# facebookresearch/fast3r

Hardware: AMD Instinct MI355X
Metric: views/sec (512^2, ViT-L) single forward pass at N=320 (higher is better)
Workload: dtype fp16

## Files before the change

fast3r_amd/csrc/f3r_gemm.hip:

```cpp
#include <stdlib.h>

#include "f3r_common.h"
#include "f3r_gemm_epi.h"

namespace {

constexpr int BM = 128, BN = 128, BK = 64, NT = 256;
constexpr int TILE_ELEMS = 128 * 64;
constexpr int GEMM_LDS_BYTES = 2 * 2 * TILE_ELEMS * 2;

__device__ __forceinline__ int swz(int row, int chunk) { return row * 64 + ((chunk ^ ((row >> 1) & 7)) << 3); }

struct ConvRow {
  int b, oy, ox;
  bool ok;
};

template <class T, int A_MODE, int EPI, int GLDS>
__global__ __launch_bounds__(NT, 2) void gemm_kernel(const f3r_gemm_args p) {
  extern __shared__ __attribute__((aligned(16))) uint16_t smem[];
  uint16_t* As = smem;
  uint16_t* Ws = smem + 2 * TILE_ELEMS;

  const int tid = threadIdx.x;
  const int lane = tid & 63;
  const int wid = __builtin_amdgcn_readfirstlane(tid >> 6);
  const int wm = wid >> 1, wn = wid & 1;

  const int n_tiles_n = (p.N + BN - 1) / BN;
  const int64_t n_tiles_m = (p.M + BM - 1) / BM;
  const int64_t n_wg = n_tiles_m * n_tiles_n;
  int64_t wg = blockIdx.x;
  {
    const int64_t q = n_wg / 8, r = n_wg % 8;
    const int64_t xcd = wg % 8, idx = wg / 8;
    wg = (xcd < r ? xcd * (q + 1) : r * (q + 1) + (xcd - r) * q) + idx;
  }
  constexpr int GM = 8;
  const int64_t per_group = (int64_t)GM * n_tiles_n;
  const int64_t grp = wg / per_group;
  const int64_t first_m = grp * GM;
  const int gm = (int)((n_tiles_m - first_m) < GM ? (n_tiles_m - first_m) : GM);
  const int64_t rem_ = wg - grp * per_group;
  const int tn = (int)(rem_ / gm);
  const int64_t tm = first_m + rem_ % gm;
  const int64_t m0 = tm * BM;
  const int n0 = tn * BN;

  const int sc = tid & 7;
  const int sr0 = tid >> 3;
  const uint16_t* Ag = (const uint16_t*)p.A;
  const uint16_t* Wg = (const uint16_t*)p.W;

  ConvRow cr[4];
  int64_t a_row_off[4];
  bool a_row_ok[4];
  bool w_row_ok[4];
  int64_t w_row_off[4];
#pragma unroll
  for (int i = 0; i < 4; ++i) {
    const int64_t m = m0 + sr0 + 32 * i;
    a_row_ok[i] = m < p.M;
    if (A_MODE == F3R_A_PLAIN) {
      a_row_off[i] = m * p.lda;
    } else {
      const int64_t per_img = (int64_t)p.conv_OH * p.conv_OW;
      const int64_t mm = a_row_ok[i] ? m : 0;
      cr[i].b = (int)(mm / per_img);
      const int rem = (int)(mm % per_img);
      cr[i].oy = rem / p.conv_OW;
      cr[i].ox = rem % p.conv_OW;
      cr[i].ok = a_row_ok[i];
      a_row_off[i] = 0;
    }
    const int n = n0 + sr0 + 32 * i;
    w_row_ok[i] = n < p.N;
    w_row_off[i] = (int64_t)n * p.Kpad;
  }

  const int nseg = p.split == F3R_SPLIT_NONE ? 1 : (p.split == F3R_SPLIT_W2 ? 2 : 3);
  const int Kpad1 = p.split == F3R_SPLIT_NONE ? p.Kpad : p.Kpad / 2;
  const int nk1 = Kpad1 / BK;
  const int nk = nseg * nk1;
  const int cpad_tiles = (A_MODE == F3R_A_CONV3X3) ? ((p.conv_C + 63) / 64) : 1;
  const uint16_t* Alo = (const uint16_t*)p.A_lo;

  u32x4 ra[4], rw[4];
  auto load_tile = [&](int kt_all) {
    const int seg = kt_all / nk1;
    const int kt = kt_all - seg * nk1;
    const uint16_t* Ag = (seg == 2) ? Alo : (const uint16_t*)p.A;
    if (A_MODE == F3R_A_PLAIN) {
      const int k = kt * BK + sc * 8;
      const bool kok = (k + 8) <= p.K;
#pragma unroll
      for (int i = 0; i < 4; ++i) {
        u32x4 v = {0u, 0u, 0u, 0u};
        if (a_row_ok[i] && kok) v = *(const u32x4*)(Ag + a_row_off[i] + k);
        ra[i] = v;
      }
    } else {
      const int tap = kt / cpad_tiles;
      const int ci = (kt - tap * cpad_tiles) * 64 + sc * 8;
      const int dy = tap / 3 - 1, dx = tap % 3 - 1;
      const bool cok = ci < p.conv_C;
#pragma unroll
      for (int i = 0; i < 4; ++i) {
        const int iy = cr[i].oy * p.conv_stride + dy;
        const int ix = cr[i].ox * p.conv_stride + dx;
        u32x4 v = {0u, 0u, 0u, 0u};
        if (cr[i].ok && cok && iy >= 0 && iy < p.conv_H && ix >= 0 && ix < p.conv_W) {
          const int64_t off = (((int64_t)cr[i].b * p.conv_H + iy) * p.conv_W + ix) * p.conv_C + ci;
          v = *(const u32x4*)(Ag + off);
          if (p.a_relu) {
            v[0] = relu_pk(v[0]);
            v[1] = relu_pk(v[1]);
            v[2] = relu_pk(v[2]);
            v[3] = relu_pk(v[3]);
          }
        }
        ra[i] = v;
      }
    }
    const int kw = (seg == 1 ? Kpad1 : 0) + kt * BK + sc * 8;
#pragma unroll
    for (int i = 0; i < 4; ++i) {
      u32x4 v = {0u, 0u, 0u, 0u};
      if (w_row_ok[i]) v = *(const u32x4*)(Wg + w_row_off[i] + kw);
      rw[i] = v;
    }
  };
  auto store_tile = [&](int buf) {
    uint16_t* a = As + buf * TILE_ELEMS;
    uint16_t* w = Ws + buf * TILE_ELEMS;
#pragma unroll
    for (int i = 0; i < 4; ++i) {
      const int r = sr0 + 32 * i;
      *(u32x4*)(a + swz(r, sc)) = ra[i];
      *(u32x4*)(w + swz(r, sc)) = rw[i];
    }
  };

  float4v acc[4][4];
#pragma unroll
  for (int i = 0; i < 4; ++i)
#pragma unroll
    for (int j = 0; j < 4; ++j) acc[i][j] = float4v{0.f, 0.f, 0.f, 0.f};

  const int Dq_ = p.qkv_dq ? p.qkv_dq : p.N / 3;
  const bool swap_roles = (EPI == F3R_EPI_QKV) && (n0 + wn * 64 >= Dq_ + (p.N - Dq_) / 2);

  const int fr = lane & 15;
  const int fg = lane >> 4;

  const int offA = (swap_roles ? 0 : 2 * TILE_ELEMS);
  const int offB = (swap_roles ? 2 * TILE_ELEMS : 0);
  const int rowA = (swap_roles ? wm : wn) * 64 + fr;
  const int rowB = (swap_roles ? wn : wm) * 64 + fr;

  auto compute = [&](int buf) {
    const uint16_t* ta = smem + offA + buf * TILE_ELEMS;
    const uint16_t* tb = smem + offB + buf * TILE_ELEMS;
#pragma unroll
    for (int ks = 0; ks < 2; ++ks) {
      typename T::vec8 fa[4], fb[4];
#pragma unroll
      for (int f = 0; f < 4; ++f) {
        fa[f] = as_vec8<T>(*(const u32x4*)(ta + swz(rowA + f * 16, ks * 4 + fg)));
        fb[f] = as_vec8<T>(*(const u32x4*)(tb + swz(rowB + f * 16, ks * 4 + fg)));
      }
#pragma unroll
      for (int i = 0; i < 4; ++i)
#pragma unroll
        for (int j = 0; j < 4; ++j) acc[i][j] = T::mfma16(fa[i], fb[j], acc[i][j]);
    }
  };

  if constexpr (GLDS == 1) {
    typedef __attribute__((address_space(3))) void* lds_ptr_t;
    typedef const __attribute__((address_space(1))) void* glb_ptr_t;
    const int lrow = lane >> 3, pch = lane & 7;
    const uint16_t* asrc[4];
    const uint16_t* wsrc[4];
#pragma unroll
    for (int i = 0; i < 4; ++i) {
      const int r = (wid * 4 + i) * 8 + lrow;
      const int lch = pch ^ ((r >> 1) & 7);
      int64_t m = m0 + r;
      if (m >= p.M) m = p.M - 1;
      int n = n0 + r;
      if (n >= p.N) n = p.N - 1;
      asrc[i] = Ag + m * p.lda + lch * 8;
      wsrc[i] = Wg + (int64_t)n * p.Kpad + lch * 8;
    }
    const int64_t alo_delta = Alo ? (Alo - Ag) : 0;
    auto dma_tile = [&](int kt_all, int buf) {
      const int seg = kt_all / nk1;
      const int kt = kt_all - seg * nk1;
      const int64_t ka = (seg == 2 ? alo_delta : 0) + (int64_t)kt * BK;
      const int kw = (seg == 1 ? Kpad1 : 0) + kt * BK;
#pragma unroll
      for (int i = 0; i < 4; ++i) {
        uint16_t* la = As + buf * TILE_ELEMS + (wid * 4 + i) * 8 * 64;
        uint16_t* lw = Ws + buf * TILE_ELEMS + (wid * 4 + i) * 8 * 64;
        __builtin_amdgcn_global_load_lds((glb_ptr_t)(asrc[i] + ka), (lds_ptr_t)la, 16, 0, 0);
        __builtin_amdgcn_global_load_lds((glb_ptr_t)(wsrc[i] + kw), (lds_ptr_t)lw, 16, 0, 0);
      }
    };
    dma_tile(0, 0);
    __syncthreads();
    int cur = 0;
    for (int kt = 0; kt < nk; ++kt) {
      if (kt + 1 < nk) dma_tile(kt + 1, cur ^ 1);
      compute(cur);
      __syncthreads();
      cur ^= 1;
    }
  } else {
    load_tile(0);
    store_tile(0);
    __syncthreads();
    int cur = 0;
    for (int kt = 0; kt < nk; ++kt) {
      const bool more = (kt + 1) < nk;
      if (more) load_tile(kt + 1);
      compute(cur);
      if (more) store_tile(cur ^ 1);
      __syncthreads();
      cur ^= 1;
    }
  }

  const int64_t m_base = m0 + wm * 64;
  const int n_base = n0 + wn * 64;
  if (swap_roles) gemm_epilogue_vt<T, GemmFragLayout<4, 4, 4, 4>, true>(p, &acc[0][0], m_base, n_base, lane);
  else gemm_epilogue_default<T, EPI, GemmFragLayout<4, 4, 4, 4>, true>(p, &acc[0][0], m_base, n_base, lane);
}

template <class T, int A_MODE, int EPI, int GLDS>
int launch(const f3r_gemm_args& a, hipStream_t stream) {
  static bool attr_set = false;
  auto kern = gemm_kernel<T, A_MODE, EPI, GLDS>;
  if (!attr_set) {
    (void)hipFuncSetAttribute((const void*)kern, hipFuncAttributeMaxDynamicSharedMemorySize, GEMM_LDS_BYTES);
    attr_set = true;
  }
  const int64_t tiles = ((a.M + BM - 1) / BM) * ((a.N + BN - 1) / BN);
  if (tiles <= 0) return F3R_OK;
  F3R_REQUIRE(tiles < (1ll << 31), "f3r_gemm: grid too large");
  hipLaunchKernelGGL(kern, dim3((unsigned)tiles), dim3(NT), GEMM_LDS_BYTES, stream, a);
  return f3r_check_launch("f3r_gemm");
}

template <class T>
int dispatch(const f3r_gemm_args& a, hipStream_t stream) {
  if (a.a_mode == F3R_A_CONV3X3) return launch<T, F3R_A_CONV3X3, F3R_EPI_GENERIC, 0>(a, stream);
  const int Kpad1 = a.split ? a.Kpad / 2 : a.Kpad;
  const bool glds = a.K == Kpad1 && a.M > 0;
  switch (a.epi) {
    case F3R_EPI_GENERIC: return glds ? launch<T, F3R_A_PLAIN, F3R_EPI_GENERIC, 1>(a, stream) : launch<T, F3R_A_PLAIN, F3R_EPI_GENERIC, 0>(a, stream);
    case F3R_EPI_QKV: return glds ? launch<T, F3R_A_PLAIN, F3R_EPI_QKV, 1>(a, stream) : launch<T, F3R_A_PLAIN, F3R_EPI_QKV, 0>(a, stream);
    case F3R_EPI_CONVT: return launch<T, F3R_A_PLAIN, F3R_EPI_CONVT, 0>(a, stream);
  }
  f3r_set_error("f3r_gemm: bad epi %d", a.epi);
  return F3R_ERR_ARG;
}

inline bool al16(const void* p) { return (((uintptr_t)p) & 15) == 0; }
inline bool al8(const void* p) { return (((uintptr_t)p) & 7) == 0; }

}

extern "C" int f3r_gemm(const f3r_gemm_args* args, f3r_stream_t stream) {
  F3R_REQUIRE(args != nullptr, "f3r_gemm: null args");
  const f3r_gemm_args& a = *args;
  F3R_REQUIRE(a.A && a.W, "f3r_gemm: null operand");
  F3R_REQUIRE(a.M >= 0 && a.N > 0, "f3r_gemm: bad M/N (%lld, %d)", (long long)a.M, a.N);
  F3R_REQUIRE(a.split >= F3R_SPLIT_NONE && a.split <= F3R_SPLIT_X3F8, "f3r_gemm: bad split %d", a.split);
  if (a.split == F3R_SPLIT_W2F8) {
    F3R_REQUIRE(al16(a.A) && al16(a.W) && a.w_scale && (((uintptr_t)a.w_scale) & 3) == 0, "f3r_gemm: W2F8 needs 16-byte aligned A / W and w_scale");
    F3R_REQUIRE(a.K > 0 && a.K % 128 == 0 && a.Kpad == a.K, "f3r_gemm: W2F8 needs K = Kpad, a multiple of 128 (got %d / %d)", a.K, a.Kpad);
    F3R_REQUIRE(a.lda % 8 == 0 && a.lda * 2 >= (int64_t)a.K * 3, "f3r_gemm: W2F8 rows are [K fp16 | K fp8]: lda %lld must be >= 3 K / 2", (long long)a.lda);
    F3R_REQUIRE(a.epi != F3R_EPI_GENERIC || a.out_f32 || a.out_lp, "f3r_gemm: no output");
    F3R_REQUIRE(!a.out_f8 && !a.out_relu_f8 && !a.fin_w, "f3r_gemm: W2F8 launches write one output (no out_f8 / out_relu_f8 / fin_w)");
    F3R_REQUIRE((a.kernel_sel >= 0 && a.kernel_sel <= 7) || a.kernel_sel == 9, "f3r_gemm: bad kernel_sel %d", a.kernel_sel);
    F3R_REQUIRE(a.dtype == F3R_F16, "f3r_gemm: W2F8 corrects fp16 planes only (dtype %d)", a.dtype);
    F3R_REQUIRE(a.act >= F3R_ACT_NONE && a.act <= F3R_ACT_RELU, "f3r_gemm: bad act %d", a.act);
    F3R_REQUIRE(a.N % 4 == 0 && (!a.bias || al16(a.bias)), "f3r_gemm: N %d must be a multiple of 4, bias 16-byte aligned", a.N);
    if (a.epi == F3R_EPI_GENERIC) {
      F3R_REQUIRE(!a.out_f32 || (al16(a.out_f32) && a.ldo_f32 % 4 == 0 && a.ldo_f32 >= a.N), "f3r_gemm: out_f32 alignment/ld");
      F3R_REQUIRE(!a.out_lp || (al16(a.out_lp) && a.ldo_lp % 8 == 0 && a.ldo_lp >= a.N), "f3r_gemm: out_lp alignment/ld");
      F3R_REQUIRE(!a.res_f32 || (al16(a.res_f32) && a.ldr_f32 % 4 == 0 && a.ldr_f32 >= a.N), "f3r_gemm: res_f32 alignment/ld");
    }
    const char* why = "";
    if (a.epi == F3R_EPI_QKV) {
      F3R_REQUIRE(a.qkv_dq != 0 || a.N % 3 == 0, "f3r_gemm: QKV with three equal parts needs N %% 3 == 0 (got %d)", a.N);
      {
        const int Dq = a.qkv_dq ? a.qkv_dq : a.N / 3;
        F3R_REQUIRE(Dq > 0 && Dq % 64 == 0 && a.N > Dq && (a.N - Dq) % 128 == 0, "f3r_gemm: QKV parts must be whole 64-wide heads (N %d, q %d)", a.N, Dq);
      }
      F3R_REQUIRE(a.q && a.k && a.vt && a.W_aux && al16(a.W_aux) && a.seq_len > 0 && a.M % a.seq_len == 0 && a.ldvt >= a.seq_len && a.act == F3R_ACT_NONE,
                  "f3r_gemm: W2F8 QKV needs q, k, vt, W_aux (16-byte aligned), seq_len dividing M, no activation");
      if (a.rope_cos) F3R_REQUIRE(a.rope_sin && a.rope_w > 0 && al16(a.rope_cos) && al16(a.rope_sin), "f3r_gemm: RoPE tables");
      if (!f3r_gemm_asm_qkv_eligible(a, &why)) {
        f3r_set_error("f3r_gemm: split W2F8 QKV but the launch is not eligible for the hand-scheduled kernel: %s", why);
        return F3R_ERR_UNSUPPORTED;
      }
      return f3r_gemm_asm_qkv_launch(a, (hipStream_t)stream);
    }
    if (!f3r_gemm_asm_f8_eligible(a, &why)) {
      f3r_set_error("f3r_gemm: split W2F8 (fp8 low plane) but the launch is not eligible for the hand-scheduled kernel: %s", why);
      return F3R_ERR_UNSUPPORTED;
    }
    return f3r_gemm_asm_f8_launch(a, (hipStream_t)stream);
  }
  F3R_REQUIRE(a.epi == F3R_EPI_GENERIC || (!a.out_f8 && !a.out_relu_f8 && !a.fin_w), "f3r_gemm: out_f8 / out_relu_f8 / fin_w need the generic epilogue (epi %d)", a.epi);
  const int planes = a.split ? 2 : 1;
  F3R_REQUIRE(a.Kpad > 0 && a.Kpad % (64 * planes) == 0, "f3r_gemm: Kpad %d must be a positive multiple of %d", a.Kpad, 64 * planes);
  const int Kpad1 = a.Kpad / planes;
  F3R_REQUIRE((a.split != F3R_SPLIT_X3 && a.split != F3R_SPLIT_X3F8) || (a.A_lo && al16(a.A_lo) && !a.a_relu), "f3r_gemm: X3 / X3F8 split needs A_lo (16-byte aligned) and no a_relu");
  if (a.split == F3R_SPLIT_X3F8)
    F3R_REQUIRE(a.a_mode == F3R_A_CONV3X3 && a.dtype == F3R_F16 && a.conv_C % 128 == 0 && a.w_scale && (((uintptr_t)a.w_scale) & 3) == 0,
                "f3r_gemm: X3F8 needs a 3x3 convolution with conv_C %% 128 == 0 (got %d), fp16 planes and w_scale", a.conv_C);
  F3R_REQUIRE((a.kernel_sel >= 0 && a.kernel_sel <= 7) || a.kernel_sel == 9 || a.kernel_sel >= 16, "f3r_gemm: bad kernel_sel %d", a.kernel_sel);
  F3R_REQUIRE(a.N % 4 == 0, "f3r_gemm: N %d must be a multiple of 4", a.N);
  F3R_REQUIRE(al16(a.A) && al16(a.W), "f3r_gemm: A/W must be 16-byte aligned");
  F3R_REQUIRE(a.dtype == F3R_F16 || a.dtype == F3R_BF16, "f3r_gemm: bad dtype %d", a.dtype);
  if (a.a_mode == F3R_A_PLAIN) {
    F3R_REQUIRE(a.K > 0 && a.K % 8 == 0 && a.K <= Kpad1, "f3r_gemm: K %d must be a multiple of 8 and <= Kpad", a.K);
    F3R_REQUIRE(a.lda % 8 == 0 && a.lda >= a.K, "f3r_gemm: lda %lld must be a multiple of 8 and >= K", (long long)a.lda);
  } else if (a.a_mode == F3R_A_CONV3X3) {
    F3R_REQUIRE(a.conv_C > 0 && a.conv_C % 8 == 0, "f3r_gemm: conv_C %d must be a multiple of 8", a.conv_C);
    F3R_REQUIRE(Kpad1 == 9 * ((a.conv_C + 63) / 64) * 64, "f3r_gemm: conv Kpad %d != 9*roundup(C,64) per plane", a.Kpad);
    F3R_REQUIRE(a.epi == F3R_EPI_GENERIC, "f3r_gemm: conv3x3 supports only the generic epilogue");
    F3R_REQUIRE(a.conv_stride == 1 || a.conv_stride == 2, "f3r_gemm: conv stride %d", a.conv_stride);
    F3R_REQUIRE(a.conv_OH == (a.conv_H + 2 - 3) / a.conv_stride + 1 && a.conv_OW == (a.conv_W + 2 - 3) / a.conv_stride + 1,
                "f3r_gemm: conv output dims inconsistent");
    F3R_REQUIRE(a.conv_OH > 0 && a.conv_OW > 0 && a.M % ((int64_t)a.conv_OH * a.conv_OW) == 0, "f3r_gemm: conv M not a multiple of OH*OW");
  } else {
    f3r_set_error("f3r_gemm: bad a_mode %d", a.a_mode);
    return F3R_ERR_ARG;
  }
  if (a.epi == F3R_EPI_GENERIC) {
    F3R_REQUIRE(a.out_f32 || a.out_lp || a.fin_w, "f3r_gemm: no output");
    F3R_REQUIRE(!a.out_f32 || (al16(a.out_f32) && a.ldo_f32 % 4 == 0 && a.ldo_f32 >= a.N), "f3r_gemm: out_f32 alignment/ld");
    F3R_REQUIRE(!a.out_lp || (al8(a.out_lp) && a.ldo_lp % 4 == 0 && a.ldo_lp >= a.N), "f3r_gemm: out_lp alignment/ld");
    F3R_REQUIRE((!a.out_f8 && !a.out_relu_f8) || (a.dtype == F3R_F16 && a.N % 8 == 0 && al8(a.out_f8) && al8(a.out_relu_f8) && !a.out_lp_f8),
                "f3r_gemm: out_f8 / out_relu_f8 need fp16, N %% 8 == 0 and 8-byte aligned buffers");
    if (a.fin_w) {
      F3R_REQUIRE(a.fin_b && a.fin_pts && al16(a.fin_w) && (a.fin_n_out == 3 || a.fin_n_out == 4) && (a.fin_n_out == 4 || !a.fin_conf),
                  "f3r_gemm: fin_w needs fin_b, fin_pts, a 16-byte aligned [4][N] weight and fin_n_out 3 or 4 (a confidence output needs 4)");
      F3R_REQUIRE(a.fin_depth_mode >= 0 && a.fin_depth_mode <= 2 && (a.fin_conf_mode == 0 || a.fin_conf_mode == 1), "f3r_gemm: bad fin_depth_mode / fin_conf_mode");
      F3R_REQUIRE(!a.out_f32 && !a.out_relu && !a.out_f8 && !a.out_relu_f8 && !a.res_lp && !a.res_f32 && !a.rowadd,
                  "f3r_gemm: the fused head tail writes fin_pts / fin_conf only");
    }
    F3R_REQUIRE(!a.res_f32 || (al16(a.res_f32) && a.ldr_f32 % 4 == 0), "f3r_gemm: res_f32 alignment/ld");
    F3R_REQUIRE(!a.res_lp || (al8(a.res_lp) && a.ldr_lp % 4 == 0), "f3r_gemm: res_lp alignment/ld");
    F3R_REQUIRE(!a.res_lp2 || (al8(a.res_lp2) && a.ldr_lp2 % 4 == 0), "f3r_gemm: res_lp2 alignment/ld");
    F3R_REQUIRE((!a.res_lp_lo || (a.res_lp && al8(a.res_lp_lo))) && (!a.res_lp2_lo || (a.res_lp2 && al8(a.res_lp2_lo))), "f3r_gemm: low residual planes need their high planes");
    F3R_REQUIRE((!a.out_lp_lo || (a.out_lp && al8(a.out_lp_lo))) && (!a.out_relu || (al8(a.out_relu) && a.ldo_lp % 4 == 0 && a.ldo_lp >= a.N)) &&
                (!a.out_relu_lo || (a.out_relu && al8(a.out_relu_lo))), "f3r_gemm: out_lp_lo / out_relu alignment");
    F3R_REQUIRE(!a.rowadd || (al16(a.rowadd) && a.rowadd_div > 0), "f3r_gemm: rowadd alignment/div");
    const int64_t ld_max = 1ll << 26;
    F3R_REQUIRE((!a.out_f32 || a.ldo_f32 < ld_max) && (!a.out_lp || a.ldo_lp < ld_max) && (!a.res_f32 || (a.ldr_f32 >= 0 && a.ldr_f32 < ld_max)) &&
                (!a.res_lp || (a.ldr_lp >= 0 && a.ldr_lp < ld_max)) && (!a.res_lp2 || (a.ldr_lp2 >= 0 && a.ldr_lp2 < ld_max)), "f3r_gemm: row strides must be < 2^26 elements");
    F3R_REQUIRE(!a.bias || al16(a.bias), "f3r_gemm: bias alignment");
  } else if (a.epi == F3R_EPI_QKV) {
    const int Dq = a.qkv_dq ? a.qkv_dq : a.N / 3;
    F3R_REQUIRE(a.qkv_dq != 0 || a.N % 3 == 0, "f3r_gemm: QKV with three equal parts needs N %% 3 == 0 (got %d)", a.N);
    F3R_REQUIRE(Dq > 0 && Dq % 64 == 0 && a.N > Dq && (a.N - Dq) % 128 == 0, "f3r_gemm: QKV parts must be whole 64-wide heads (N %d, q %d)", a.N, Dq);
    F3R_REQUIRE(a.q && a.k && a.vt && al8(a.q) && al8(a.k) && al8(a.vt), "f3r_gemm: QKV outputs null/misaligned");
    F3R_REQUIRE(a.seq_len > 0 && a.M % a.seq_len == 0 && a.ldvt >= a.seq_len, "f3r_gemm: QKV seq_len/ldvt");
    F3R_REQUIRE(a.act == F3R_ACT_NONE, "f3r_gemm: QKV has no activation");
    F3R_REQUIRE(!a.bias || al16(a.bias), "f3r_gemm: bias alignment");
    if (a.rope_cos) F3R_REQUIRE(a.rope_sin && a.rope_w > 0 && al16(a.rope_cos) && al16(a.rope_sin), "f3r_gemm: RoPE tables");
  } else if (a.epi == F3R_EPI_CONVT) {
    F3R_REQUIRE(a.out_lp && al8(a.out_lp), "f3r_gemm: CONVT needs out_lp");
    F3R_REQUIRE(a.ct_s > 0 && a.ct_cout > 0 && a.ct_cout % 4 == 0 && a.N == a.ct_s * a.ct_s * a.ct_cout, "f3r_gemm: CONVT N != s*s*cout");
    F3R_REQUIRE(a.ct_h > 0 && a.ct_w > 0 && a.M % ((int64_t)a.ct_h * a.ct_w) == 0, "f3r_gemm: CONVT M not a multiple of h*w");
    F3R_REQUIRE(!a.bias || al16(a.bias), "f3r_gemm: bias alignment");
  }
  hipStream_t s = (hipStream_t)stream;
  if (a.kernel_sel >= 16) return f3r_gemm256_lab(a, s);
  if (a.split == F3R_SPLIT_X3F8 || a.fin_w) {
    if (!f3r_gemm256_eligible(a)) {
      f3r_set_error("f3r_gemm: split X3F8 / fin_w but the launch is not eligible for the 256-tile kernel (conv_C %% 64 (X3F8: 128) == 0, "
                    "N %% 128 == 0 (fin_w: N == 128), operand below 4 GiB)");
      return F3R_ERR_UNSUPPORTED;
    }
    return f3r_gemm256_launch(a, s, 1);
  }
  if (a.kernel_sel == 6 || a.kernel_sel == 0 || a.kernel_sel == 9) {
    const char* why = "";
    if (a.epi == F3R_EPI_QKV && f3r_gemm_asm_qkv_eligible(a, &why) && (a.kernel_sel == 6 || a.kernel_sel == 9 || f3r_gemm_asm_preferred((a.M / 256) * (a.N / 3 / 256))))
      return f3r_gemm_asm_qkv_launch(a, s);
    const bool ok = a.epi != F3R_EPI_QKV && f3r_gemm_asm_eligible(a, &why);
    if ((a.kernel_sel == 6 || a.kernel_sel == 9) && !ok) {
      f3r_set_error("f3r_gemm: kernel_sel 6 (hand-scheduled kernel) but the launch is not eligible: %s", why);
      return F3R_ERR_UNSUPPORTED;
    }
    if (ok && (a.kernel_sel == 6 || a.kernel_sel == 9 || f3r_gemm_asm_preferred((a.M / 256) * (a.N / 256)))) return f3r_gemm_asm_launch(a, s);
  }
  const int sel = a.kernel_sel == 7 ? 0 : a.kernel_sel;
  if (sel >= 2) F3R_REQUIRE(f3r_gemm256_eligible(a), "f3r_gemm: kernel_sel %d but the shape is not eligible for the 256-tile kernel", sel);
  if (sel >= 2 || (sel == 0 && f3r_gemm256_eligible(a) && f3r_gemm256_preferred(a))) return f3r_gemm256_launch(a, s, sel != 3);
  return a.dtype == F3R_F16 ? dispatch<F16>(a, s) : dispatch<BF16>(a, s);
}
```

fast3r_amd/csrc/f3r_gemm256.hip:

```cpp
#include "f3r_gemm256_impl.h"

int f3r_gemm256_run_bf16(const f3r_gemm_args& a, hipStream_t stream, int stagger);
int f3r_gemm256_run_conv_f8_fin(const f3r_gemm_args& a, hipStream_t stream);

bool f3r_gemm256_eligible(const f3r_gemm_args& a) {
  if (a.N % 128 != 0) return false;
  if (a.epi == F3R_EPI_QKV) {
    const int Dq = a.qkv_dq ? a.qkv_dq : a.N / 3;
    if (Dq % 256 != 0 || ((a.N - Dq) / 2) % 256 != 0) return false;
  }
  const int Kpad1 = a.split ? a.Kpad / 2 : a.Kpad;
  if (Kpad1 % 64 != 0) return false;
  if (a.a_mode == F3R_A_PLAIN) {
    if (a.K != Kpad1) return false;
    if ((int64_t)256 * a.lda * 2 >= (1ll << 32)) return false;
  } else {
    if (a.a_relu || a.conv_C % 64 != 0) return false;
    if (a.M / ((int64_t)a.conv_OH * a.conv_OW) * a.conv_H * a.conv_W * a.conv_C * 2 >= (1ll << 32)) return false;
    if (a.split == F3R_SPLIT_X3F8 && (a.conv_C % 128 != 0 || a.dtype != F3R_F16)) return false;
  }
  if (a.split == F3R_SPLIT_X3F8 && a.a_mode != F3R_A_CONV3X3) return false;
  if (a.fin_w && (a.a_mode != F3R_A_CONV3X3 || a.N != 128 || a.epi != F3R_EPI_GENERIC)) return false;
  if ((int64_t)256 * a.Kpad * 2 >= (1ll << 32)) return false;
  const int add = gemm_additive_pattern(a);
  if (add == F3R_ADD_UNSUPPORTED || (add != F3R_ADD_NONE && a.act != F3R_ACT_NONE)) return false;
  if (add != F3R_ADD_NONE && a.epi != F3R_EPI_GENERIC) return false;
  if (a.a_mode == F3R_A_CONV3X3 ? (add == F3R_ADD_RES_F32 || add == F3R_ADD_ROWADD) : add == F3R_ADD_RES_LP) return false;
  return true;
}

bool f3r_gemm256_preferred(const f3r_gemm_args& a) { return score_256(a, tile_halves(a)) >= score_128(a); }

int f3r_gemm256_launch(const f3r_gemm_args& a, hipStream_t stream, int stagger) {
  const int64_t tiles = ((a.M + BM - 1) / BM) * ((a.N + 127) / 128);
  if (tiles <= 0) return F3R_OK;
  F3R_REQUIRE(tiles < (1ll << 31), "f3r_gemm: grid too large");
  if (a.split == F3R_SPLIT_X3F8 || a.fin_w) return f3r_gemm256_run_conv_f8_fin(a, stream);
  return a.dtype == F3R_F16 ? dispatch256<F16>(a, stream, stagger) : f3r_gemm256_run_bf16(a, stream, stagger);
}
```

fast3r_amd/csrc/f3r_gemm256_f8.hip:

```cpp
#include <cstdlib>

#include "f3r_gemm256_impl.h"

int f3r_gemm256_run_conv_f8_fin(const f3r_gemm_args& a, hipStream_t stream) {
  const bool f8 = a.split == F3R_SPLIT_X3F8;
  const int add = gemm_additive_pattern(a);
  if (a.fin_w) {
#ifdef F3R_CONV_ABLATIONS
    if (f8) {
      static const char* ab = getenv("F3R_CONV_ABLATE");
      switch (ab ? atoi(ab) : 0) {
#define F3R_ABL(n) case n: return launch256<F16, F3R_A_CONV3X3, F3R_EPI_GENERIC, 1, F3R_ADD_NONE, 1, true, true, false, n>(a, stream);
        F3R_ABL(1) F3R_ABL(1024) F3R_ABL(2048) F3R_ABL(2) F3R_ABL(4) F3R_ABL(3) F3R_ABL(7)
#undef F3R_ABL
      }
    }
#endif
    if (a.dtype == F3R_BF16) return launch256<BF16, F3R_A_CONV3X3, F3R_EPI_GENERIC, 1, F3R_ADD_NONE, 1, false, true>(a, stream);
    if (f8 && a.kernel_sel == 5) return launch256<F16, F3R_A_CONV3X3, F3R_EPI_GENERIC, 1, F3R_ADD_NONE, 1, true, true, true>(a, stream);
    return f8 ? launch256<F16, F3R_A_CONV3X3, F3R_EPI_GENERIC, 1, F3R_ADD_NONE, 1, true, true>(a, stream)
              : launch256<F16, F3R_A_CONV3X3, F3R_EPI_GENERIC, 1, F3R_ADD_NONE, 1, false, true>(a, stream);
  }
  const int nh = tile_halves(a);
  if (add == F3R_ADD_RES_LP)
    return nh == 2 ? launch256<F16, F3R_A_CONV3X3, F3R_EPI_GENERIC, 1, F3R_ADD_RES_LP, 2, true>(a, stream)
                   : launch256<F16, F3R_A_CONV3X3, F3R_EPI_GENERIC, 1, F3R_ADD_RES_LP, 1, true>(a, stream);
  return nh == 2 ? launch256<F16, F3R_A_CONV3X3, F3R_EPI_GENERIC, 1, F3R_ADD_NONE, 2, true>(a, stream)
                 : launch256<F16, F3R_A_CONV3X3, F3R_EPI_GENERIC, 1, F3R_ADD_NONE, 1, true>(a, stream);
}
```

fast3r_amd/csrc/f3r_gemm256_impl.h:

```cpp
#pragma once
#include <atomic>

#include "f3r_common.h"
#include "f3r_gemm_epi.h"


namespace {

constexpr int BM = 256, BK = 64, NT = 512;
constexpr int HT = 128 * 64;
template <int NH> struct TileCfg {
  static constexpr int BN = 128 * NH;
  static constexpr int BUF = (2 + NH) * HT;
  static constexpr int NBUF = NH == 2 ? 2 : 3;
  static constexpr int TAB_ENTRIES = 512;
  static constexpr int LDS_BYTES = NBUF * BUF * 2 + TAB_ENTRIES * 16;
};

inline int f3r_num_cus() {
  constexpr int MAXD = 64;
  static std::atomic<int> cache[MAXD];
  int dev = 0;
  if (hipGetDevice(&dev) != hipSuccess) dev = 0;
  if (dev >= 0 && dev < MAXD) {
    const int c = cache[dev].load(std::memory_order_relaxed);
    if (c) return c;
  }
  int cu = 0;
  if (hipDeviceGetAttribute(&cu, hipDeviceAttributeMultiprocessorCount, dev) != hipSuccess || cu < 8) cu = 256;
  const int n = cu / 8 * 8;
  if (dev >= 0 && dev < MAXD) cache[dev].store(n, std::memory_order_relaxed);
  return n;
}

typedef __attribute__((address_space(3))) void* lds_ptr_t;
typedef const __attribute__((address_space(1))) void* glb_ptr_t;

template <int V>
struct IC {
  static constexpr int value = V;
};

#define F3R_VMCNT(n) __builtin_amdgcn_s_waitcnt(0x0F70 | (n))
#define F3R_LGKMCNT0() __builtin_amdgcn_s_waitcnt(0xC07F)

template <class T, int A_MODE, int EPI, bool SWAP, int STAGGER, int ADDSRC, int NH = 2, int LAB = 0, bool F8 = false, bool FIN = false, bool MERGED = false>
__device__ __forceinline__ void gemm256_body(const f3r_gemm_args& p, uint16_t* smem, const int64_t m0_tile, const int n0_tile, const bool first = true,
                                             const bool has_next = false, const int64_t m0_next = 0, const int n0_next = 0) {
  constexpr int BUF = TileCfg<NH>::BUF;
  int64_t m0 = m0_tile;
  int n0 = n0_tile;
  const int tid = threadIdx.x;
  const int lane = tid & 63;
  const int wid = __builtin_amdgcn_readfirstlane(tid >> 6);
  const int wm = wid >> 2, wn = wid & 3;
  const int fr = lane & 15, fg = lane >> 4;
  constexpr bool PAIRED = EPI != F3R_EPI_QKV && (ADDSRC == F3R_ADD_NONE || ADDSRC == F3R_ADD_RES_LP);
  static_assert(!(PAIRED && SWAP), "swapped roles exist only in the QKV role");
  auto w_key = [](int r) { return PAIRED ? (((r >> 1) & 1) | (((r >> 3) & 3) << 1)) : ((r >> 1) & 7); };
  uint64_t stamp[5] = {0, 0, 0, 0, 0};
  if (LAB & 128) stamp[0] = __builtin_amdgcn_s_memtime();
  if ((LAB & (256 | 512)) && blockIdx.x < 256) {
    const int PH = (LAB & 512) ? 4 : 2;
    const int phase = (blockIdx.x >> 3) & (PH - 1);
    const int n = phase * (p.Kpad / BK) * (4 / PH);
    for (int i = 0; i < n; ++i) __builtin_amdgcn_s_sleep(15);
  }

  const int nseg = p.split == F3R_SPLIT_NONE ? 1 : (p.split == F3R_SPLIT_W2 ? 2 : 3);
  const int Kpad1 = p.split == F3R_SPLIT_NONE ? p.Kpad : p.Kpad / 2;
  const int nk1 = Kpad1 / BK;
  const int nk8 = nk1 / 2;
  const int nk = F8 ? nk1 + 2 * nk8 : nseg * nk1;
  const int ctiles = A_MODE == F3R_A_CONV3X3 ? p.conv_C / 64 : 1;
  const int ctiles8 = A_MODE == F3R_A_CONV3X3 ? p.conv_C / 128 : 1;
  static_assert(!F8 || (A_MODE == F3R_A_CONV3X3 && !SWAP), "fp8 correction segments: convolutions only");
  static_assert(!FIN || (NH == 1 && EPI == F3R_EPI_GENERIC && ADDSRC == 0 && !SWAP), "fused head tail: 256 x 128 tiles, no additive terms");

  uint32_t a_off[2][2], w_off[2][2];
  uint32_t a_msk[2][2];
  const char* const Ab = (const char*)p.A;
  const char* const Alo = (const char*)p.A_lo;
  const uint32_t a_bytes = A_MODE == F3R_A_CONV3X3 ? (uint32_t)(p.M / ((int64_t)p.conv_OH * p.conv_OW) * p.conv_H * p.conv_W * p.conv_C * 2) : 0u;
  const char* Wb = nullptr;
  uint32_t wsc[NH][2];
  auto setup_tile = [&](int64_t tm0, int tn0) {
  m0 = tm0;
  n0 = tn0;
  Wb = (const char*)p.W + (int64_t)n0 * p.Kpad * 2;
  if constexpr (F8) {
#pragma unroll
    for (int h = 0; h < NH; ++h)
#pragma unroll
      for (int nf = 0; nf < 2; ++nf) {
        int n = n0 + h * 128 + (wid & 3) * 32 + (PAIRED ? (fr >> 2) * 8 + (fr & 3) + nf * 4 : fr + nf * 16);
        if (n >= p.N) n = p.N - 1;
        wsc[h][nf] = p.w_scale[n];
      }
  }
#pragma unroll
  for (int h = 0; h < 2; ++h)
#pragma unroll
    for (int i = 0; i < 2; ++i) {
      const int r = (wid * 2 + i) * 8 + (lane >> 3);
      const int lc = (lane & 7) ^ ((r >> 1) & 7);
      int n = n0 + (h < NH ? h : 0) * 128 + r;
      if (n >= p.N) n = p.N - 1;
      w_off[h][i] = (uint32_t)(((int64_t)(n - n0) * p.Kpad + ((lane & 7) ^ w_key(r)) * 8) * 2);
      int64_t m = m0 + h * 128 + r;
      if (A_MODE == F3R_A_PLAIN) {
        if (m >= p.M) m = p.M - 1;
        a_off[h][i] = (uint32_t)(((m - m0) * p.lda + lc * 8) * 2);
        a_msk[h][i] = 0;
      } else {
        const bool ok = m < p.M;
        const int64_t per_img = (int64_t)p.conv_OH * p.conv_OW;
        const int64_t mm = ok ? m : 0;
        const int b = (int)(mm / per_img);
        const int rem = (int)(mm % per_img);
        const int oy = rem / p.conv_OW, ox = rem - oy * p.conv_OW;
        const int cy = oy * p.conv_stride, cx = ox * p.conv_stride;
        a_off[h][i] = (uint32_t)(((((int64_t)b * p.conv_H + cy) * p.conv_W + cx) * p.conv_C + lc * 8) * 2);
        uint32_t msk = 0;
#pragma unroll
        for (int tap = 0; tap < 9; ++tap) {
          const int iy = cy + tap / 3 - 1, ix = cx + tap % 3 - 1;
          if (!(ok && iy >= 0 && iy < p.conv_H && ix >= 0 && ix < p.conv_W)) msk |= 1u << tap;
        }
        a_msk[h][i] = msk;
      }
    }
  };
  setup_tile(m0_tile, n0_tile);

  constexpr bool TAB = A_MODE == F3R_A_CONV3X3;
  const int pix = TAB ? p.conv_C * 2 : 0;
  uint32_t* const tab = (uint32_t*)(smem + TileCfg<NH>::NBUF * BUF);
  if (TAB && first) {
    for (int t = tid; t < nk; t += NT) {
      int delta, meta, wso;
      if (!F8 || t < nk1) {
        const int seg = F8 ? 0 : t / nk1, kk = t - seg * nk1, tapn = kk / ctiles, ct = kk - tapn * ctiles;
        delta = ((tapn / 3 - 1) * p.conv_W + (tapn % 3 - 1)) * pix + ct * 128;
        meta = tapn | ((!F8 && seg == 2) ? 16 : 0);
        wso = ((seg == 1 ? Kpad1 : 0) + kk * BK) * 2;
      } else {
        const int u = t - nk1, s8 = u / nk8, kk = u - s8 * nk8, tapn = kk / ctiles8, ct = kk - tapn * ctiles8;
        delta = ((tapn / 3 - 1) * p.conv_W + (tapn % 3 - 1)) * pix + (s8 == 1 ? p.conv_C : 0) + ct * 128;
        meta = tapn | 16;
        wso = (s8 + 2) * Kpad1 + kk * 128;
      }
      *(u32x4*)(tab + t * 4) = u32x4{(uint32_t)delta, (uint32_t)meta, (uint32_t)wso, 0u};
    }
    __syncthreads();
  }
  u32x4 ea = {0u, 0u, 0u, 0u}, ew = ea;
  int a_seg = 0, a_kk = 0, a_t = 0;
  int w_seg = 0, w_kk = 0, w_t = 0;
  auto fetch = [&]() {
    if constexpr (TAB) {
      ea = *(const u32x4*)(tab + a_t * 4);
      ew = *(const u32x4*)(tab + w_t * 4);
    }
  };
  bool dry = false;
  auto a_advance = [&]() {
    if (a_t + 1 < nk) {
      ++a_t;
      if constexpr (!TAB) {
        ++a_kk;
        if (a_kk == nk1) { a_kk = 0; ++a_seg; }
      }
    }
  };
  auto w_advance = [&]() {
    if (w_t + 1 < nk) {
      ++w_t;
      if constexpr (!TAB) {
        ++w_kk;
        if (w_kk == nk1) { w_kk = 0; ++w_seg; }
      }
    }
  };
  bool in_loop = false;
  auto issue_a = [&](int h, int buf) {
    if (dry) return;
    if ((LAB & (1 | 2048)) && in_loop) return;
    const char* plane = (!TAB && a_seg == 2) ? Alo : Ab;
    uint16_t* dst = smem + buf * BUF + h * HT + wid * 2 * 8 * 64;
    if (A_MODE == F3R_A_PLAIN) {
      const char* base = plane + (m0 * p.lda + (int64_t)a_kk * BK) * 2;
      if (LAB & 32) {
        const __amdgpu_buffer_rsrc_t rs = __builtin_amdgcn_make_buffer_rsrc((void*)(plane + m0 * p.lda * 2), 0, 0x7fffffff, 0x00020000);
#pragma unroll
        for (int i = 0; i < 2; ++i)
          __builtin_amdgcn_raw_ptr_buffer_load_lds(rs, (lds_ptr_t)(dst + i * 8 * 64), 16, (int)a_off[h][i], a_kk * BK * 2, 0, 0);
        return;
      }
#pragma unroll
      for (int i = 0; i < 2; ++i)
        __builtin_amdgcn_global_load_lds((glb_ptr_t)(base + a_off[h][i]), (lds_ptr_t)(dst + i * 8 * 64), 16, 0, 0);
    } else {
      const int a_delta = __builtin_amdgcn_readfirstlane((int)ea[0]);
      const int meta = __builtin_amdgcn_readfirstlane((int)ea[1]);
      const int a_tap = meta & 15;
      const char* pl = (meta & 16) ? Alo : Ab;
      const __amdgpu_buffer_rsrc_t rs = __builtin_amdgcn_make_buffer_rsrc((void*)pl, 0, a_bytes, 0x00020000);
#pragma unroll
      for (int i = 0; i < 2; ++i) {
        const int32_t inv = ((int32_t)(a_msk[h][i] << (31 - a_tap))) >> 31;
        const uint32_t vo = (a_off[h][i] + (uint32_t)a_delta) | (uint32_t)inv;
        __builtin_amdgcn_raw_ptr_buffer_load_lds(rs, (lds_ptr_t)(dst + i * 8 * 64), 16, (int)vo, 0, 0, 0);
      }
    }
  };
  auto issue_w = [&](int h, int buf) {
    if (dry) return;
    if ((LAB & (1 | 1024)) && in_loop) return;
    uint16_t* dst = smem + buf * BUF + (2 + h) * HT + wid * 2 * 8 * 64;
    if constexpr (TAB) {
      const int w_soff = __builtin_amdgcn_readfirstlane((int)ew[2]);
      const __amdgpu_buffer_rsrc_t rs = __builtin_amdgcn_make_buffer_rsrc((void*)Wb, 0, 0x7fffffff, 0x00020000);
#pragma unroll
      for (int i = 0; i < 2; ++i)
        __builtin_amdgcn_raw_ptr_buffer_load_lds(rs, (lds_ptr_t)(dst + i * 8 * 64), 16, (int)w_off[h][i], w_soff, 0, 0);
      return;
    }
    const char* base = Wb + ((int64_t)(w_seg == 1 ? Kpad1 : 0) + (int64_t)w_kk * BK) * 2;
    if (LAB & 32) {
      const __amdgpu_buffer_rsrc_t rs = __builtin_amdgcn_make_buffer_rsrc((void*)Wb, 0, 0x7fffffff, 0x00020000);
#pragma unroll
      for (int i = 0; i < 2; ++i)
        __builtin_amdgcn_raw_ptr_buffer_load_lds(rs, (lds_ptr_t)(dst + i * 8 * 64), 16, (int)w_off[h][i], ((w_seg == 1 ? Kpad1 : 0) + w_kk * BK) * 2, 0, 0);
      return;
    }
#pragma unroll
    for (int i = 0; i < 2; ++i)
      __builtin_amdgcn_global_load_lds((glb_ptr_t)(base + w_off[h][i]), (lds_ptr_t)(dst + i * 8 * 64), 16, 0, 0);
  };

  const int sw = (fr >> 1) & 7;
  const int w_row = wn * 32 + (PAIRED ? (fr >> 2) * 8 + (fr & 3) : fr);
  int a_rd[2], w_rd[2];
#pragma unroll
  for (int ks = 0; ks < 2; ++ks) {
    a_rd[ks] = (wm * 64 + fr) * 64 + (((ks * 4 + fg) ^ sw) << 3);
    w_rd[ks] = w_row * 64 + (((ks * 4 + fg) ^ w_key(w_row)) << 3);
  }

  float4v acc[16 * NH];
  typename T::vec8 fa0[2][4], fa1[2][4], fw[2][2];
  typedef uint32_t u32x8 __attribute__((ext_vector_type(8)));
  typedef int i32x8 __attribute__((ext_vector_type(8)));
  u32x8 ga0[4], ga1[4], gw[2];

  auto read_a = [&](auto e8, auto which, int buf, int mh) {
    if ((LAB & 2) && in_loop) return;
    if constexpr (decltype(e8)::value) {
      auto& g = decltype(which)::value ? ga1 : ga0;
#pragma unroll
      for (int mf = 0; mf < 4; ++mf) {
        const u32x4 c0 = *(const u32x4*)(smem + buf * BUF + mh * HT + a_rd[0] + mf * 16 * 64);
        const u32x4 c1 = *(const u32x4*)(smem + buf * BUF + mh * HT + a_rd[1] + mf * 16 * 64);
        g[mf] = __builtin_shufflevector(c0, c1, 0, 1, 2, 3, 4, 5, 6, 7);
      }
    } else {
      auto& f = decltype(which)::value ? fa1 : fa0;
#pragma unroll
      for (int ks = 0; ks < 2; ++ks)
#pragma unroll
        for (int mf = 0; mf < 4; ++mf)
          f[ks][mf] = as_vec8<T>(*(const u32x4*)(smem + buf * BUF + mh * HT + a_rd[ks] + mf * 16 * 64));
    }
  };
  auto read_w = [&](auto e8, int buf, int nh) {
    if ((LAB & 2) && in_loop) return;
    if constexpr (decltype(e8)::value) {
#pragma unroll
      for (int nf = 0; nf < 2; ++nf) {
        const u32x4 c0 = *(const u32x4*)(smem + buf * BUF + (2 + nh) * HT + w_rd[0] + nf * (PAIRED ? 4 : 16) * 64);
        const u32x4 c1 = *(const u32x4*)(smem + buf * BUF + (2 + nh) * HT + w_rd[1] + nf * (PAIRED ? 4 : 16) * 64);
        gw[nf] = __builtin_shufflevector(c0, c1, 0, 1, 2, 3, 4, 5, 6, 7);
      }
    } else {
#pragma unroll
      for (int ks = 0; ks < 2; ++ks)
#pragma unroll
        for (int nf = 0; nf < 2; ++nf)
          fw[ks][nf] = as_vec8<T>(*(const u32x4*)(smem + buf * BUF + (2 + nh) * HT + w_rd[ks] + nf * (PAIRED ? 4 : 16) * 64));
    }
  };
  auto mma = [&](auto e8, auto which, int mh, int nh, int sa_shift, int sb) {
    if (LAB & 4) return;
    if constexpr (decltype(e8)::value) {
      auto& g = decltype(which)::value ? ga1 : ga0;
#pragma unroll
      for (int nf = 0; nf < 2; ++nf) {
        const int sa = (int)((wsc[nh < NH ? nh : 0][nf] >> sa_shift) & 0xffu);
#pragma unroll
        for (int mf = 0; mf < 4; ++mf) {
          const int NF = nh * 2 + nf, MF = mh * 4 + mf;
          acc[NF * 8 + MF] = __builtin_amdgcn_mfma_scale_f32_16x16x128_f8f6f4(__builtin_bit_cast(i32x8, gw[nf]), __builtin_bit_cast(i32x8, g[mf]),
                                                                              acc[NF * 8 + MF], 0, 0, 0, sa, 0, sb);
        }
      }
#pragma unroll
      for (int nf = 0; nf < 2; ++nf)
#pragma unroll
        for (int mf = 0; mf < 4; ++mf) asm volatile("" : "+v"(acc[(nh * 2 + nf) * 8 + mh * 4 + mf]));
    } else {
      auto& f = decltype(which)::value ? fa1 : fa0;
#pragma unroll
      for (int ks = 0; ks < 2; ++ks)
#pragma unroll
        for (int nf = 0; nf < 2; ++nf)
#pragma unroll
          for (int mf = 0; mf < 4; ++mf) {
            const int NF = nh * 2 + nf, MF = mh * 4 + mf;
            if (SWAP) acc[MF * (2 * NH) + NF] = T::mfma16(f[ks][mf], fw[ks][nf], acc[MF * (2 * NH) + NF]);
            else      acc[NF * 8 + MF] = T::mfma16(fw[ks][nf], f[ks][mf], acc[NF * 8 + MF]);
          }
    }
  };

#define F3R_PHASE_MMA(WHICH, MH, NH)                     \
  __builtin_amdgcn_sched_barrier(0);                     \
  __builtin_amdgcn_s_barrier();                          \
  F3R_LGKMCNT0();                                        \
  __builtin_amdgcn_sched_barrier(0);                     \
  if (!(LAB & 16)) __builtin_amdgcn_s_setprio(1);        \
  mma(e8, IC<WHICH>{}, MH, NH, sa_shift, sb);            \
  if (!(LAB & 16)) __builtin_amdgcn_s_setprio(0);        \
  __builtin_amdgcn_sched_barrier(0);                     \
  __builtin_amdgcn_s_barrier();
  auto tile = [&](auto bufc, auto e8, int sa_shift, int sb) {
    constexpr int B = decltype(bufc)::value;
    fetch();
    read_w(e8, B, 0);
    if (!(LAB & 64)) __builtin_amdgcn_sched_barrier(0);
    read_a(e8, IC<0>{}, B, 0);
    issue_a(1, B ^ 1);
    a_advance();
    if (!(LAB & 8)) F3R_VMCNT(8);
    F3R_PHASE_MMA(0, 0, 0)
    fetch();
    read_a(e8, IC<1>{}, B, 1);
    issue_w(1, B ^ 1);
    w_advance();
    if (!(LAB & 8)) F3R_VMCNT(8);
    F3R_PHASE_MMA(1, 1, 0)
    fetch();
    read_w(e8, B, 1);
    issue_a(0, B);
    F3R_PHASE_MMA(1, 1, 1)
    fetch();
    issue_w(0, B);
    if (!(LAB & 8)) F3R_VMCNT(8);
    F3R_PHASE_MMA(0, 0, 1)
  };
  auto tile1 = [&](auto bufc, auto e8, int sa_shift, int sb) {
    constexpr int B = decltype(bufc)::value;
    constexpr int B2 = (B + 2) % 3;
    fetch();
    read_w(e8, B, 0);
    if (!(LAB & 64)) __builtin_amdgcn_sched_barrier(0);
    read_a(e8, IC<0>{}, B, 0);
    issue_a(0, B2);
    issue_w(0, B2);
    w_advance();
    if (!(LAB & 8)) F3R_VMCNT(10);
    F3R_PHASE_MMA(0, 0, 0)
    read_a(e8, IC<1>{}, B, 1);
    issue_a(1, B2);
    a_advance();
    if (!(LAB & 8)) F3R_VMCNT(8);
    F3R_PHASE_MMA(1, 1, 0)
  };
#define F3R_MMA2_OPEN()                                  \
  __builtin_amdgcn_sched_barrier(0);                     \
  __builtin_amdgcn_s_barrier();                          \
  F3R_LGKMCNT0();                                        \
  __builtin_amdgcn_sched_barrier(0);                     \
  __builtin_amdgcn_s_setprio(1);
#define F3R_MMA2_ISSUE()                                 \
  __builtin_amdgcn_s_setprio(0);                         \
  __builtin_amdgcn_sched_barrier(0);
#define F3R_MMA2_CLOSE()                                 \
  __builtin_amdgcn_sched_barrier(0);                     \
  __builtin_amdgcn_s_barrier();
  auto tileM = [&](auto bufc, auto e8, int sa_shift, int sb) {
    constexpr int B = decltype(bufc)::value;
    fetch();
    read_w(e8, B, 0);
    __builtin_amdgcn_sched_barrier(0);
    read_a(e8, IC<0>{}, B, 0);
    read_a(e8, IC<1>{}, B, 1);
    issue_w(1, B ^ 1);
    w_advance();
    F3R_VMCNT(8);
    F3R_MMA2_OPEN()
    mma(e8, IC<0>{}, 0, 0, sa_shift, sb);
    mma(e8, IC<1>{}, 1, 0, sa_shift, sb);
    F3R_MMA2_ISSUE()
    F3R_MMA2_CLOSE()
    fetch();
    read_w(e8, B, 1);
    issue_a(0, B);
    issue_w(0, B);
    issue_a(1, B);
    a_advance();
    F3R_VMCNT(8);
    F3R_MMA2_OPEN()
    mma(e8, IC<1>{}, 1, 1, sa_shift, sb);
    mma(e8, IC<0>{}, 0, 1, sa_shift, sb);
    F3R_MMA2_ISSUE()
    F3R_MMA2_CLOSE()
  };
  auto tile1M = [&](auto bufc, auto e8, int sa_shift, int sb) {
    constexpr int B = decltype(bufc)::value;
    constexpr int B2 = (B + 2) % 3;
    fetch();
    read_w(e8, B, 0);
    __builtin_amdgcn_sched_barrier(0);
    read_a(e8, IC<0>{}, B, 0);
    read_a(e8, IC<1>{}, B, 1);
    issue_a(0, B2);
    issue_w(0, B2);
    w_advance();
    issue_a(1, B2);
    a_advance();
    F3R_VMCNT(6);
    F3R_MMA2_OPEN()
    mma(e8, IC<0>{}, 0, 0, sa_shift, sb);
    mma(e8, IC<1>{}, 1, 0, sa_shift, sb);
    F3R_MMA2_ISSUE()
    F3R_MMA2_CLOSE()
  };
#undef F3R_MMA2_OPEN
#undef F3R_MMA2_ISSUE
#undef F3R_MMA2_CLOSE
#undef F3R_PHASE_MMA

  typedef GemmFragLayout<2 * NH, 8, 2, 4, PAIRED> Frag;
  const int64_t m_base = m0_tile + wm * 64;
  const int n_base = n0_tile + wn * 32;
  auto opening_loads = [&]() {
    a_seg = a_kk = a_t = 0;
    w_seg = w_kk = w_t = 0;
    if constexpr (NH == 2) {
      if (!dry) fetch();
      issue_a(0, 0);
      issue_w(0, 0);
      issue_a(1, 0);
      a_advance();
      issue_w(1, 0);
      w_advance();
      if (!dry) fetch();
      issue_a(0, 1);
      issue_w(0, 1);
      if constexpr (MERGED) {
        issue_a(1, 1);
        a_advance();
      }
    } else {
      if (!dry) fetch();
      issue_a(0, 0);
      issue_w(0, 0);
      w_advance();
      issue_a(1, 0);
      a_advance();
      if (!dry) fetch();
      issue_a(0, 1);
      issue_w(0, 1);
      w_advance();
      issue_a(1, 1);
      a_advance();
    }
  };
  dry = !first;
  opening_loads();
  dry = false;
  gemm_acc_init_additive<T, Frag, ADDSRC, SWAP>(p, acc, m_base, n_base, lane);
  if (first && MERGED) {
    if constexpr (NH == 2) F3R_VMCNT(8);
    else F3R_VMCNT(6);
  } else if (first) {
    F3R_VMCNT(8);
  } else {
    F3R_VMCNT(0);
  }
  __builtin_amdgcn_s_barrier();
  if (STAGGER && wm == 1) __builtin_amdgcn_s_barrier();
  if (LAB & 128) stamp[1] = __builtin_amdgcn_s_memtime();

  typedef IC<0> E16;
  typedef IC<1> E8;
  auto T2 = [&](auto bufc, auto e8, int sa_shift, int sb) {
    if constexpr (MERGED) tileM(bufc, e8, sa_shift, sb);
    else tile(bufc, e8, sa_shift, sb);
  };
  auto T1 = [&](auto bufc, auto e8, int sa_shift, int sb) {
    if constexpr (MERGED) tile1M(bufc, e8, sa_shift, sb);
    else tile1(bufc, e8, sa_shift, sb);
  };
  const int nk16 = F8 ? nk1 : nk;
  if constexpr (NH == 2) {
    if (LAB) {
      tile(IC<0>{}, E16{}, 0, 0);
      if (nk > 1) tile(IC<1>{}, E16{}, 0, 0);
      in_loop = true;
    }
    for (int t = LAB ? 2 : 0; t < nk16; t += 2) {
      T2(IC<0>{}, E16{}, 0, 0);
      if (t + 1 < nk16) T2(IC<1>{}, E16{}, 0, 0);
    }
    if constexpr (F8) {
      for (int t = 0; t < nk1; t += 2) {
        T2(IC<0>{}, E8{}, t >= nk8 ? 8 : 0, t >= nk8 ? 115 : 127);
        T2(IC<1>{}, E8{}, t + 1 >= nk8 ? 8 : 0, t + 1 >= nk8 ? 115 : 127);
      }
    }
  } else {
    if (LAB) in_loop = true;
    for (int t = 0; t < nk16; t += 3) {
      T1(IC<0>{}, E16{}, 0, 0);
      if (t + 1 < nk16) T1(IC<1>{}, E16{}, 0, 0);
      if (t + 2 < nk16) T1(IC<2>{}, E16{}, 0, 0);
    }
    if constexpr (F8) {
      for (int t = 0; t < nk1; t += 3) {
        T1(IC<0>{}, E8{}, t >= nk8 ? 8 : 0, t >= nk8 ? 115 : 127);
        T1(IC<1>{}, E8{}, t + 1 >= nk8 ? 8 : 0, t + 1 >= nk8 ? 115 : 127);
        T1(IC<2>{}, E8{}, t + 2 >= nk8 ? 8 : 0, t + 2 >= nk8 ? 115 : 127);
      }
    }
  }
  F3R_VMCNT(0);
  if (STAGGER && wm == 0) __builtin_amdgcn_s_barrier();
  if (LAB & 128) stamp[2] = __builtin_amdgcn_s_memtime();
  if (has_next) {
    setup_tile(m0_next, n0_next);
    opening_loads();
  }

  if constexpr (FIN) {
    __builtin_amdgcn_s_barrier();
    gemm_epilogue_fin<T, Frag>(p, acc, m0_tile, wm, wn, lane, tid, (float*)(smem + 2 * BUF));
  } else if (SWAP) gemm_epilogue_vt<T, Frag, false>(p, acc, m_base, n_base, lane);
  else gemm_epilogue_default<T, EPI, Frag, false>(p, acc, m_base, n_base, lane);
  if (LAB & 128) {
    __builtin_amdgcn_sched_barrier(0);
    stamp[3] = __builtin_amdgcn_s_memtime();
    F3R_VMCNT(0);
    stamp[4] = __builtin_amdgcn_s_memtime();
    if (tid == 0) {
      uint64_t* d = (uint64_t*)p.rope_cos + (int64_t)blockIdx.x * 5;
      for (int i = 0; i < 5; ++i) d[i] = stamp[i];
    }
  }
}

template <class T, int A_MODE, int EPI, int STAGGER, int ADDSRC, int NH, bool F8 = false, bool FIN = false, bool MERGED = false, int LAB = 0>
__global__ __launch_bounds__(NT, 1) void gemm256_kernel(const f3r_gemm_args p) {
  extern __shared__ __attribute__((aligned(16))) uint16_t smem[];
  constexpr int BN = TileCfg<NH>::BN;
  const int n_tiles_n = (p.N + BN - 1) / BN;
  const int64_t n_tiles_m = (p.M + BM - 1) / BM;
  const int64_t n_wg = n_tiles_m * n_tiles_n;
  auto tile_of = [&](int64_t wg, int64_t& m0, int& n0) {
    {
      const int64_t q = n_wg / 8, r = n_wg % 8;
      const int64_t xcd = wg % 8, idx = wg / 8;
      wg = (xcd < r ? xcd * (q + 1) : r * (q + 1) + (xcd - r) * q) + idx;
    }
    constexpr int GM = 8;
    const int64_t per_group = (int64_t)GM * n_tiles_n;
    const int64_t grp = wg / per_group;
    const int64_t first_m = grp * GM;
    const int gm = (int)((n_tiles_m - first_m) < GM ? (n_tiles_m - first_m) : GM);
    const int64_t rem_ = wg - grp * per_group;
    const int tn = (int)(rem_ / gm);
    const int64_t tm = first_m + rem_ % gm;
    m0 = tm * BM;
    n0 = tn * BN;
  };
  int64_t m0, m0n = 0;
  int n0, n0n = 0;
  bool first = true;
  for (int64_t v = blockIdx.x; v < n_wg; v += gridDim.x) {
    tile_of(v, m0, n0);
    const bool has_next = v + gridDim.x < n_wg;
    if (has_next) tile_of(v + gridDim.x, m0n, n0n);
    bool done = false;
    if constexpr (EPI == F3R_EPI_QKV) {
      if (n0 >= (p.qkv_dq ? p.qkv_dq + (p.N - p.qkv_dq) / 2 : 2 * (p.N / 3))) {
        gemm256_body<T, A_MODE, EPI, true, STAGGER, F3R_ADD_NONE, NH>(p, smem, m0, n0, first, has_next, m0n, n0n);
        done = true;
      }
    }
    if (!done) gemm256_body<T, A_MODE, EPI, false, STAGGER, ADDSRC, NH, LAB, F8, FIN, MERGED>(p, smem, m0, n0, first, has_next, m0n, n0n);
    first = false;
  }
}

template <class T, int A_MODE, int EPI, int STAGGER, int ADDSRC, int NH, bool F8 = false, bool FIN = false, bool MERGED = false, int LAB = 0>
int launch256(const f3r_gemm_args& a, hipStream_t stream) {
  static bool attr_set = false;
  auto kern = gemm256_kernel<T, A_MODE, EPI, STAGGER, ADDSRC, NH, F8, FIN, MERGED, LAB>;
  constexpr int LDS_BYTES = TileCfg<NH>::LDS_BYTES, BN = TileCfg<NH>::BN;
  if (!attr_set) {
    (void)hipFuncSetAttribute((const void*)kern, hipFuncAttributeMaxDynamicSharedMemorySize, LDS_BYTES);
    attr_set = true;
  }
  const int64_t tiles = ((a.M + BM - 1) / BM) * ((a.N + BN - 1) / BN);
  const int64_t grid = (a.kernel_sel == 5 || tiles <= f3r_num_cus()) ? tiles : f3r_num_cus();
  hipLaunchKernelGGL(kern, dim3((unsigned)grid), dim3(NT), LDS_BYTES, stream, a);
  return f3r_check_launch("f3r_gemm(256)");
}

inline float tile_score(int64_t tiles, int slots, float eff) {
  if (tiles <= 0) return 0.f;
  const int64_t rounds = (tiles + slots - 1) / slots;
  return eff * (float)tiles / (float)(rounds * slots);
}
inline float score_256(const f3r_gemm_args& a, int nh) {
  return tile_score(((a.M + 255) / 256) * ((a.N + 128 * nh - 1) / (128 * nh)), 256, nh == 2 ? 1.0f : 0.82f);
}
inline float score_128(const f3r_gemm_args& a) { return tile_score(((a.M + 127) / 128) * ((a.N + 127) / 128), 512, 0.72f); }

inline int tile_halves(const f3r_gemm_args& a) {
  if (a.epi == F3R_EPI_QKV) return 2;
  if (a.N % 256 != 0 || a.kernel_sel == 4) return 1;
  if (a.kernel_sel == 2 || a.kernel_sel == 3 || a.kernel_sel == 5) return 2;
  return score_256(a, 1) > score_256(a, 2) ? 1 : 2;
}

template <class T>
int dispatch256(const f3r_gemm_args& a, hipStream_t stream, int stagger) {
#define F3R_L256H(AM, EP, AD, NHV) (stagger ? launch256<T, AM, EP, 1, AD, NHV>(a, stream) : launch256<T, AM, EP, 0, AD, NHV>(a, stream))
#define F3R_L256(AM, EP, AD) (nh == 2 ? F3R_L256H(AM, EP, AD, 2) : F3R_L256H(AM, EP, AD, 1))
  const int add = gemm_additive_pattern(a);
  const int nh = tile_halves(a);
  if (a.a_mode == F3R_A_CONV3X3) return add == F3R_ADD_RES_LP ? F3R_L256(F3R_A_CONV3X3, F3R_EPI_GENERIC, F3R_ADD_RES_LP) : F3R_L256(F3R_A_CONV3X3, F3R_EPI_GENERIC, F3R_ADD_NONE);
  switch (a.epi) {
    case F3R_EPI_GENERIC:
      return add == F3R_ADD_RES_F32 ? F3R_L256(F3R_A_PLAIN, F3R_EPI_GENERIC, F3R_ADD_RES_F32)
           : add == F3R_ADD_ROWADD ? F3R_L256(F3R_A_PLAIN, F3R_EPI_GENERIC, F3R_ADD_ROWADD) : F3R_L256(F3R_A_PLAIN, F3R_EPI_GENERIC, F3R_ADD_NONE);
    case F3R_EPI_QKV: return F3R_L256H(F3R_A_PLAIN, F3R_EPI_QKV, F3R_ADD_NONE, 2);
    default: return F3R_L256(F3R_A_PLAIN, F3R_EPI_CONVT, F3R_ADD_NONE);
  }
#undef F3R_L256
#undef F3R_L256H
}

#ifdef F3R_GEMM_LAB
template <class T, int LAB>
__global__ __launch_bounds__(NT, 1) void gemm256_lab_kernel(const f3r_gemm_args p) {
  extern __shared__ __attribute__((aligned(16))) uint16_t smem[];
  constexpr int BN = 256;
  const int n_tiles_n = (p.N + BN - 1) / BN;
  const int64_t wg = blockIdx.x;
  gemm256_body<T, F3R_A_PLAIN, F3R_EPI_GENERIC, false, 1, F3R_ADD_NONE, 2, LAB>(p, smem, (wg / n_tiles_n) * BM, (int)(wg % n_tiles_n) * BN);
}
template <class T, int LAB>
int launch_lab(const f3r_gemm_args& a, hipStream_t stream) {
  auto kern = gemm256_lab_kernel<T, LAB>;
  constexpr int BN = 256, LDS_BYTES = TileCfg<2>::LDS_BYTES;
  (void)hipFuncSetAttribute((const void*)kern, hipFuncAttributeMaxDynamicSharedMemorySize, LDS_BYTES);
  const int64_t tiles = ((a.M + BM - 1) / BM) * ((a.N + BN - 1) / BN);
  hipLaunchKernelGGL(kern, dim3((unsigned)tiles), dim3(NT), LDS_BYTES, stream, a);
  return f3r_check_launch("f3r_gemm(256 lab)");
}
#endif

}
```

fast3r_amd/csrc/f3r_gemm_epi.h:

```cpp
#pragma once
#include "f3r_common.h"

template <int NF_, int MF_, int NG_, int MG_, bool PAIRED_ = false>
struct GemmFragLayout {
  static constexpr int NF = NF_, MF = MF_, NG = NG_, MG = MG_;
  static constexpr bool PAIRED = PAIRED_;
  static constexpr int LW = PAIRED_ ? 8 : 4;
  static constexpr int STEP = PAIRED_ ? 2 : 1;
  static_assert(!PAIRED_ || NG_ == 2, "paired columns: two fragments per 32-column group");
  static __device__ __forceinline__ int row(int mf) { return (mf / MG) * 128 + (mf % MG) * 16; }
  static __device__ __forceinline__ int col(int nf) { return (nf / NG) * 128 + (nf % NG) * (PAIRED_ ? 4 : 16); }
  static __device__ __forceinline__ int col_end() { return ((NF - 1) / NG) * 128 + NG * 16; }
};

__device__ __forceinline__ float gelu_erf(float x) {
  const float z = fabsf(x) * 0.70710678118654752440f;
  const float t = __builtin_amdgcn_rcpf(__builtin_fmaf(0.3275911f, z, 1.0f));
  float poly = __builtin_fmaf(1.061405429f, t, -1.453152027f);
  poly = __builtin_fmaf(poly, t, 1.421413741f);
  poly = __builtin_fmaf(poly, t, -0.284496736f);
  poly = __builtin_fmaf(poly, t, 0.254829592f);
  const float u = poly * t * __builtin_amdgcn_exp2f(-z * z * 1.44269504088896340736f);
  const float h = 0.5f * x * u;
  return x >= 0.f ? x - h : h;
}

__device__ __forceinline__ float4v gelu_erf4(float4v x) {
  float4v t, e;
#pragma unroll
  for (int i = 0; i < 4; ++i) t[i] = __builtin_amdgcn_rcpf(__builtin_fmaf(__builtin_fabsf(x[i]), 0.3275911f * 0.70710678118654752440f, 1.0f));
  float4v poly = t * (0.5f * 1.061405429f) + (0.5f * -1.453152027f);
  poly = poly * t + (0.5f * 1.421413741f);
  poly = poly * t + (0.5f * -0.284496736f);
  poly = poly * t + (0.5f * 0.254829592f);
  const float4v arg = (x * x) * (-0.5f * 1.44269504088896340736f);
#pragma unroll
  for (int i = 0; i < 4; ++i) e[i] = __builtin_amdgcn_exp2f(arg[i]);
  const float4v h = x * (poly * t * e);
  float4v r;
#pragma unroll
  for (int i = 0; i < 4; ++i) r[i] = __builtin_fmaf(x[i] + __builtin_fabsf(x[i]), 0.5f, -__builtin_fabsf(h[i]));
  return r;
}

template <class T>
__device__ __forceinline__ void store4_split(uint16_t* hi, uint16_t* lo, float4v v) {
  u32x2 o;
  o[0] = pack2<T>(v[0], v[1]);
  o[1] = pack2<T>(v[2], v[3]);
  *(u32x2*)hi = o;
  if (lo) {
    u32x2 r;
    r[0] = pack2<T>(v[0] - lo_f<T>(o[0]), v[1] - hi_f<T>(o[0]));
    r[1] = pack2<T>(v[2] - lo_f<T>(o[1]), v[3] - hi_f<T>(o[1]));
    *(u32x2*)lo = r;
  }
}

template <class T>
__device__ __forceinline__ float4v load4_lp(const uint16_t* ptr) {
  const u32x2 r = *(const u32x2*)ptr;
  return float4v{lo_f<T>(r[0]), hi_f<T>(r[0]), lo_f<T>(r[1]), hi_f<T>(r[1])};
}

template <class T, int STEP>
__device__ __forceinline__ void storeN_split(char* hi, char* lo, const float4v* v) {
  if constexpr (STEP == 1) {
    store4_split<T>((uint16_t*)hi, (uint16_t*)lo, v[0]);
  } else {
    u32x4 o;
    o[0] = pack2<T>(v[0][0], v[0][1]); o[1] = pack2<T>(v[0][2], v[0][3]);
    o[2] = pack2<T>(v[1][0], v[1][1]); o[3] = pack2<T>(v[1][2], v[1][3]);
    *(u32x4*)hi = o;
    if (lo) {
      u32x4 r;
      r[0] = pack2<T>(v[0][0] - lo_f<T>(o[0]), v[0][1] - hi_f<T>(o[0])); r[1] = pack2<T>(v[0][2] - lo_f<T>(o[1]), v[0][3] - hi_f<T>(o[1]));
      r[2] = pack2<T>(v[1][0] - lo_f<T>(o[2]), v[1][1] - hi_f<T>(o[2])); r[3] = pack2<T>(v[1][2] - lo_f<T>(o[3]), v[1][3] - hi_f<T>(o[3]));
      *(u32x4*)lo = r;
    }
  }
}
template <class T, int STEP>
__device__ __forceinline__ void loadN_lp(const char* ptr, float4v* v) {
  if constexpr (STEP == 1) {
    v[0] = load4_lp<T>((const uint16_t*)ptr);
  } else {
    const u32x4 r = *(const u32x4*)ptr;
    v[0] = float4v{lo_f<T>(r[0]), hi_f<T>(r[0]), lo_f<T>(r[1]), hi_f<T>(r[1])};
    v[1] = float4v{lo_f<T>(r[2]), hi_f<T>(r[2]), lo_f<T>(r[3]), hi_f<T>(r[3])};
  }
}

__device__ __forceinline__ uint32_t f8x4(float a, float b, float c, float d) {
  auto cl = [](float x) { return fminf(fmaxf(x, -448.f), 448.f); };
  int w = __builtin_amdgcn_cvt_pk_fp8_f32(cl(a), cl(b), 0, false);
  w = __builtin_amdgcn_cvt_pk_fp8_f32(cl(c), cl(d), w, true);
  return (uint32_t)w;
}
__device__ __forceinline__ float f16_rest(float x) { return (x - (float)(_Float16)x) * 4096.f; }
template <int STEP>
__device__ __forceinline__ void storeN_f8(char* hi8, char* lo8, const float4v* v) {
  if constexpr (STEP == 1) {
    *(uint32_t*)hi8 = f8x4(v[0][0], v[0][1], v[0][2], v[0][3]);
    *(uint32_t*)lo8 = f8x4(f16_rest(v[0][0]), f16_rest(v[0][1]), f16_rest(v[0][2]), f16_rest(v[0][3]));
  } else {
    u32x2 h, l;
    h[0] = f8x4(v[0][0], v[0][1], v[0][2], v[0][3]);
    h[1] = f8x4(v[1][0], v[1][1], v[1][2], v[1][3]);
    l[0] = f8x4(f16_rest(v[0][0]), f16_rest(v[0][1]), f16_rest(v[0][2]), f16_rest(v[0][3]));
    l[1] = f8x4(f16_rest(v[1][0]), f16_rest(v[1][1]), f16_rest(v[1][2]), f16_rest(v[1][3]));
    *(u32x2*)hi8 = h;
    *(u32x2*)lo8 = l;
  }
}

template <class T, int NF, int MB, class F>
__device__ __forceinline__ void gemm_additive_terms(const f3r_gemm_args& p, const int64_t (&mc)[MB], const int (&nbc)[NF], F&& term) {
  if (p.rowadd) {
#pragma unroll
    for (int i = 0; i < MB; ++i) {
      const float* row = p.rowadd + (mc[i] / p.rowadd_div) * (int64_t)p.N;
#pragma unroll
      for (int nf = 0; nf < NF; ++nf) term(i, nf, *(const float4v*)(row + nbc[nf]));
    }
  }
  if (p.res_f32) {
#pragma unroll
    for (int i = 0; i < MB; ++i)
#pragma unroll
      for (int nf = 0; nf < NF; ++nf) term(i, nf, *(const float4v*)(p.res_f32 + mc[i] * p.ldr_f32 + nbc[nf]));
  }
  if (p.res_lp) {
#pragma unroll
    for (int i = 0; i < MB; ++i)
#pragma unroll
      for (int nf = 0; nf < NF; ++nf) term(i, nf, load4_lp<T>((const uint16_t*)p.res_lp + mc[i] * p.ldr_lp + nbc[nf]));
    if (p.res_lp_lo) {
#pragma unroll
      for (int i = 0; i < MB; ++i)
#pragma unroll
        for (int nf = 0; nf < NF; ++nf) term(i, nf, load4_lp<T>((const uint16_t*)p.res_lp_lo + mc[i] * p.ldr_lp + nbc[nf]));
    }
  }
  if (p.res_lp2) {
#pragma unroll
    for (int i = 0; i < MB; ++i)
#pragma unroll
      for (int nf = 0; nf < NF; ++nf) term(i, nf, load4_lp<T>((const uint16_t*)p.res_lp2 + mc[i] * p.ldr_lp2 + nbc[nf]));
    if (p.res_lp2_lo) {
#pragma unroll
      for (int i = 0; i < MB; ++i)
#pragma unroll
        for (int nf = 0; nf < NF; ++nf) term(i, nf, load4_lp<T>((const uint16_t*)p.res_lp2_lo + mc[i] * p.ldr_lp2 + nbc[nf]));
    }
  }
}

enum { F3R_ADD_NONE = 0, F3R_ADD_RES_F32 = 1, F3R_ADD_ROWADD = 2, F3R_ADD_RES_LP = 3, F3R_ADD_UNSUPPORTED = -1 };

inline int gemm_additive_pattern(const f3r_gemm_args& a) {
  const int n_kinds = (a.rowadd != nullptr) + (a.res_f32 != nullptr) + (a.res_lp != nullptr || a.res_lp2 != nullptr);
  if (n_kinds == 0) return F3R_ADD_NONE;
  if (n_kinds > 1 || (a.res_lp2 && !a.res_lp)) return F3R_ADD_UNSUPPORTED;
  return a.rowadd ? F3R_ADD_ROWADD : (a.res_f32 ? F3R_ADD_RES_F32 : F3R_ADD_RES_LP);
}

template <class T, class L, int SRC, bool SWAP>
__device__ __forceinline__ void gemm_acc_init_additive(const f3r_gemm_args& p, float4v* acc, int64_t m_base, int n_base, int lane) {
  constexpr int NF = L::NF, MF = L::MF;
  const int fr = lane & 15, fg = lane >> 4;
  if (SWAP) {
#pragma unroll
    for (int nf = 0; nf < NF; ++nf) {
      const int n = n_base + L::col(nf) + fr;
      const float b = (p.bias && n < p.N) ? p.bias[n] : 0.f;
#pragma unroll
      for (int mf = 0; mf < MF; ++mf) acc[mf * NF + nf] = float4v{b, b, b, b};
    }
    return;
  }
  if (SRC != F3R_ADD_ROWADD && m_base + L::row(MF - 1) + 16 <= p.M && n_base + L::col_end() <= p.N) {
    float4v b4[NF];
#pragma unroll
    for (int nf = 0; nf < NF; ++nf)
      b4[nf] = p.bias ? *(const float4v*)((const char*)(p.bias + n_base + L::col(nf)) + (uint32_t)(fg * L::LW * 4)) : float4v{0.f, 0.f, 0.f, 0.f};
    if (SRC == F3R_ADD_NONE) {
#pragma unroll
      for (int nf = 0; nf < NF; ++nf)
#pragma unroll
        for (int mf = 0; mf < MF; ++mf) acc[nf * MF + mf] = b4[nf];
      return;
    }
    if (SRC == F3R_ADD_RES_F32) {
      const uint32_t off = (uint32_t)(fr * (int)p.ldr_f32 + fg * L::LW) * 4u;
#pragma unroll
      for (int mf = 0; mf < MF; ++mf) {
        const char* const row = (const char*)p.res_f32 + ((m_base + L::row(mf)) * p.ldr_f32 + n_base) * 4;
#pragma unroll
        for (int nf = 0; nf < NF; ++nf) acc[nf * MF + mf] = *(const float4v*)(row + L::col(nf) * 4 + off);
      }
    } else {
      const uint32_t off = (uint32_t)(fr * (int)p.ldr_lp + fg * L::LW) * 2u;
      const uint32_t off2 = (uint32_t)(fr * (int)p.ldr_lp2 + fg * L::LW) * 2u;
#pragma unroll
      for (int mf = 0; mf < MF; ++mf) {
        const int64_t ro = ((m_base + L::row(mf)) * p.ldr_lp + n_base) * 2;
#pragma unroll
        for (int nf = 0; nf < NF; nf += L::STEP) {
          float4v t[L::STEP];
          loadN_lp<T, L::STEP>((const char*)p.res_lp + ro + L::col(nf) * 2 + off, t);
#pragma unroll
          for (int q = 0; q < L::STEP; ++q) acc[(nf + q) * MF + mf] = t[q];
        }
      }
      if (p.res_lp_lo) {
#pragma unroll
        for (int mf = 0; mf < MF; ++mf) {
          const int64_t ro = ((m_base + L::row(mf)) * p.ldr_lp + n_base) * 2;
#pragma unroll
          for (int nf = 0; nf < NF; nf += L::STEP) {
            float4v t[L::STEP];
            loadN_lp<T, L::STEP>((const char*)p.res_lp_lo + ro + L::col(nf) * 2 + off, t);
#pragma unroll
            for (int q = 0; q < L::STEP; ++q) acc[(nf + q) * MF + mf] += t[q];
          }
        }
      }
      if (p.res_lp2) {
#pragma unroll
        for (int mf = 0; mf < MF; ++mf) {
          const int64_t ro = ((m_base + L::row(mf)) * p.ldr_lp2 + n_base) * 2;
#pragma unroll
          for (int nf = 0; nf < NF; nf += L::STEP) {
            float4v t[L::STEP];
            loadN_lp<T, L::STEP>((const char*)p.res_lp2 + ro + L::col(nf) * 2 + off2, t);
#pragma unroll
            for (int q = 0; q < L::STEP; ++q) acc[(nf + q) * MF + mf] += t[q];
          }
        }
        if (p.res_lp2_lo) {
#pragma unroll
          for (int mf = 0; mf < MF; ++mf) {
            const int64_t ro = ((m_base + L::row(mf)) * p.ldr_lp2 + n_base) * 2;
#pragma unroll
            for (int nf = 0; nf < NF; nf += L::STEP) {
            float4v t[L::STEP];
            loadN_lp<T, L::STEP>((const char*)p.res_lp2_lo + ro + L::col(nf) * 2 + off2, t);
#pragma unroll
            for (int q = 0; q < L::STEP; ++q) acc[(nf + q) * MF + mf] += t[q];
          }
          }
        }
      }
    }
#pragma unroll
    for (int nf = 0; nf < NF; ++nf)
#pragma unroll
      for (int mf = 0; mf < MF; ++mf) acc[nf * MF + mf] += b4[nf];
    return;
  }
  int nbc[NF];
  float4v bias4[NF];
#pragma unroll
  for (int nf = 0; nf < NF; ++nf) {
    const int nb = n_base + L::col(nf) + fg * L::LW;
    nbc[nf] = nb < p.N ? nb : p.N - 4;
    bias4[nf] = p.bias ? *(const float4v*)(p.bias + nbc[nf]) : float4v{0.f, 0.f, 0.f, 0.f};
  }
  if (SRC == F3R_ADD_NONE) {
#pragma unroll
    for (int nf = 0; nf < NF; ++nf)
#pragma unroll
      for (int mf = 0; mf < MF; ++mf) acc[nf * MF + mf] = bias4[nf];
    return;
  }
  int64_t mc[MF];
#pragma unroll
  for (int mf = 0; mf < MF; ++mf) {
    const int64_t m = m_base + L::row(mf) + fr;
    mc[mf] = m < p.M ? m : p.M - 1;
  }
  if (SRC == F3R_ADD_RES_F32) {
#pragma unroll
    for (int mf = 0; mf < MF; ++mf)
#pragma unroll
      for (int nf = 0; nf < NF; ++nf) acc[nf * MF + mf] = *(const float4v*)(p.res_f32 + mc[mf] * p.ldr_f32 + nbc[nf]);
  } else if (SRC == F3R_ADD_ROWADD) {
#pragma unroll
    for (int mf = 0; mf < MF; ++mf) {
      const float* row = p.rowadd + (mc[mf] / p.rowadd_div) * (int64_t)p.N;
#pragma unroll
      for (int nf = 0; nf < NF; ++nf) acc[nf * MF + mf] = *(const float4v*)(row + nbc[nf]);
    }
  } else {
#pragma unroll
    for (int mf = 0; mf < MF; ++mf)
#pragma unroll
      for (int nf = 0; nf < NF; ++nf) acc[nf * MF + mf] = load4_lp<T>((const uint16_t*)p.res_lp + mc[mf] * p.ldr_lp + nbc[nf]);
    if (p.res_lp_lo) {
#pragma unroll
      for (int mf = 0; mf < MF; ++mf)
#pragma unroll
        for (int nf = 0; nf < NF; ++nf) acc[nf * MF + mf] += load4_lp<T>((const uint16_t*)p.res_lp_lo + mc[mf] * p.ldr_lp + nbc[nf]);
    }
    if (p.res_lp2) {
#pragma unroll
      for (int mf = 0; mf < MF; ++mf)
#pragma unroll
        for (int nf = 0; nf < NF; ++nf) acc[nf * MF + mf] += load4_lp<T>((const uint16_t*)p.res_lp2 + mc[mf] * p.ldr_lp2 + nbc[nf]);
      if (p.res_lp2_lo) {
#pragma unroll
        for (int mf = 0; mf < MF; ++mf)
#pragma unroll
          for (int nf = 0; nf < NF; ++nf) acc[nf * MF + mf] += load4_lp<T>((const uint16_t*)p.res_lp2_lo + mc[mf] * p.ldr_lp2 + nbc[nf]);
      }
    }
  }
#pragma unroll
  for (int nf = 0; nf < NF; ++nf)
#pragma unroll
    for (int mf = 0; mf < MF; ++mf) acc[nf * MF + mf] += bias4[nf];
}

#define F3R_EPI_WAIT_LOADS() __builtin_amdgcn_s_waitcnt(0x0F70)

template <class L>
__device__ __forceinline__ bool gemm_wave_interior(const f3r_gemm_args& p, int64_t m_base, int n_base) {
  return m_base + L::row(L::MF - 1) + 16 <= p.M && n_base + L::col_end() <= p.N;
}

template <int V>
struct EpiC {
  static constexpr int value = V;
};

template <class T, class L>
__device__ __forceinline__ void gemm_epilogue_generic_interior(const f3r_gemm_args& p, const float4v* acc, int64_t m_base, int n_base, int lane) {
  constexpr int NF = L::NF, MF = L::MF;
  const int fr = lane & 15, fg = lane >> 4;
  const uint32_t off_f32 = (uint32_t)(fr * (int)p.ldo_f32 + fg * L::LW) * 4u;
  const uint32_t off_lp = (uint32_t)(fr * (int)p.ldo_lp + fg * L::LW) * 2u;
  const uint32_t off_f8 = (uint32_t)(fr * p.N * 2 + fg * L::LW);
  const bool relu = p.act == F3R_ACT_RELU;
  auto run = [&](auto act_c, auto kind_c) {
    constexpr int ACT = decltype(act_c)::value, KIND = decltype(kind_c)::value;
#pragma unroll
    for (int mf = 0; mf < MF; ++mf) {
      const int64_t mrow = m_base + L::row(mf);
      char* const bf = (KIND >= 2 && p.out_f32) ? (char*)p.out_f32 + (mrow * p.ldo_f32 + n_base) * 4 : nullptr;
      const int64_t lp_row = (mrow * p.ldo_lp + n_base) * 2;
      char* const bl = (KIND != 2 && p.out_lp) ? (char*)p.out_lp + lp_row : nullptr;
      char* const bll = ((KIND == 1 || KIND == 3) && p.out_lp_lo) ? (char*)p.out_lp_lo + lp_row : nullptr;
      char* const br = (KIND == 3 && p.out_relu) ? (char*)p.out_relu + lp_row : nullptr;
      char* const brl = (KIND == 3 && p.out_relu_lo) ? (char*)p.out_relu_lo + lp_row : nullptr;
      char* const b8 = (KIND == 3 && p.out_f8) ? (char*)p.out_f8 + (mrow * p.N * 2 + n_base) : nullptr;
      char* const br8 = (KIND == 3 && p.out_relu_f8) ? (char*)p.out_relu_f8 + (mrow * p.N * 2 + n_base) : nullptr;
#pragma unroll
      for (int nf = 0; nf < NF; nf += L::STEP) {
        float4v v[L::STEP];
#pragma unroll
        for (int q = 0; q < L::STEP; ++q) {
          v[q] = acc[(nf + q) * MF + mf];
          if (ACT == F3R_ACT_GELU) v[q] = gelu_erf4(v[q]);
          else if (relu) v[q] = float4v{fmaxf(v[q][0], 0.f), fmaxf(v[q][1], 0.f), fmaxf(v[q][2], 0.f), fmaxf(v[q][3], 0.f)};
        }
        const int cb = L::col(nf);
        if (KIND >= 2 && bf) {
#pragma unroll
          for (int q = 0; q < L::STEP; ++q) *(float4v*)(bf + (cb + q * 4) * 4 + off_f32) = v[q];
        }
        if (KIND != 2 && bl) storeN_split<T, L::STEP>(bl + cb * 2 + off_lp, (KIND == 1 || (KIND == 3 && bll)) ? bll + cb * 2 + off_lp : nullptr, v);
        if (KIND == 3 && b8) storeN_f8<L::STEP>(b8 + cb + off_f8, b8 + cb + off_f8 + p.N, v);
        if (KIND == 3 && (br || br8)) {
          float4v r[L::STEP];
#pragma unroll
          for (int q = 0; q < L::STEP; ++q) r[q] = float4v{fmaxf(v[q][0], 0.f), fmaxf(v[q][1], 0.f), fmaxf(v[q][2], 0.f), fmaxf(v[q][3], 0.f)};
          if (br) storeN_split<T, L::STEP>(br + cb * 2 + off_lp, brl ? brl + cb * 2 + off_lp : nullptr, r);
          if (br8) storeN_f8<L::STEP>(br8 + cb + off_f8, br8 + cb + off_f8 + p.N, r);
        }
      }
    }
  };
  auto by_kind = [&](auto act_c) {
    const bool f32 = p.out_f32 != nullptr, lp = p.out_lp != nullptr, lo = p.out_lp_lo != nullptr, rl = p.out_relu != nullptr || p.out_f8 != nullptr || p.out_relu_f8 != nullptr;
    if (lp && !f32 && !lo && !rl) run(act_c, EpiC<0>{});
    else if (lp && lo && !f32 && !rl) run(act_c, EpiC<1>{});
    else if (f32 && !lp && !rl) run(act_c, EpiC<2>{});
    else run(act_c, EpiC<3>{});
  };
  if (p.act == F3R_ACT_GELU) by_kind(EpiC<F3R_ACT_GELU>{});
  else by_kind(EpiC<F3R_ACT_NONE>{});
}

template <class T, class L>
__device__ __forceinline__ void gemm_epilogue_qk_interior(const f3r_gemm_args& p, const float4v* acc, int64_t m_base, int n_base, int lane) {
  constexpr int NF = L::NF, MF = L::MF, MB = 4;
  const int fr = lane & 15, fg = lane >> 4;
  const int Dq = p.qkv_dq ? p.qkv_dq : p.N / 3;
  const int Dkv = (p.N - Dq) / 2;
  const int part = n_base < Dq ? 0 : 1;
  const int Dm = part == 0 ? Dq : Dkv;
  const int col0 = part == 0 ? 0 : Dq;
  char* const dst = (char*)(part == 0 ? p.q : p.k);
  const float qs = (part == 0 && p.q_scale != 0.f) ? p.q_scale : 1.f;
  const uint32_t off = (uint32_t)(fr * Dm + fg * L::LW) * 2u;
  const uint32_t seq = (uint32_t)p.seq_len, rw = (uint32_t)(p.rope_w > 0 ? p.rope_w : 1);
#pragma unroll
  for (int mb = 0; mb < MF; mb += MB) {
    float4v c[MB][NF / 2], sn[MB][NF / 2];
    if (p.rope_cos) {
#pragma unroll
      for (int i = 0; i < MB; ++i) {
        const uint32_t m = (uint32_t)(m_base + L::row(mb + i)) + (uint32_t)fr;
        const uint32_t pos = m % seq;
        const uint32_t py = pos / rw, px = pos - py * rw;
        const uint32_t grp = m / rw;
#pragma unroll
        for (int j = 0; j < NF / 2; ++j) {
          const int h = ((n_base + L::col(2 * j)) >> 5) & 1;
          const int64_t toff = p.rope_mode == 1 ? (int64_t)grp * 32 + h * 16 : (int64_t)(h == 0 ? py : px) * 16;
          c[i][j] = *(const float4v*)(p.rope_cos + toff + fg * 4);
          sn[i][j] = *(const float4v*)(p.rope_sin + toff + fg * 4);
        }
      }
      F3R_EPI_WAIT_LOADS();
    }
#pragma unroll
    for (int i = 0; i < MB; ++i) {
      char* const row = dst + ((m_base + L::row(mb + i)) * Dm + (n_base - col0)) * 2;
      float4v v[NF];
#pragma unroll
      for (int nf = 0; nf < NF; ++nf) v[nf] = acc[nf * MF + mb + i];
      if (p.rope_cos) {
#pragma unroll
        for (int j = 0; j < NF / 2; ++j) {
          const float4v a = v[2 * j], b = v[2 * j + 1];
          v[2 * j] = a * c[i][j] - b * sn[i][j];
          v[2 * j + 1] = b * c[i][j] + a * sn[i][j];
        }
      }
#pragma unroll
      for (int nf = 0; nf < NF; ++nf) store4_split<T>((uint16_t*)(row + L::col(nf) * 2 + off), nullptr, v[nf] * qs);
    }
  }
}

template <class T, int EPI, class L, bool ADD>
__device__ __forceinline__ void gemm_epilogue_default(const f3r_gemm_args& p, const float4v* acc, int64_t m_base, int n_base, int lane) {
  constexpr int NF = L::NF, MF = L::MF;
  if constexpr (!ADD && EPI != F3R_EPI_CONVT) {
    if (gemm_wave_interior<L>(p, m_base, n_base) && p.M <= 0x7fffffffll) {
      if constexpr (EPI == F3R_EPI_GENERIC) gemm_epilogue_generic_interior<T, L>(p, acc, m_base, n_base, lane);
      else gemm_epilogue_qk_interior<T, L>(p, acc, m_base, n_base, lane);
      return;
    }
  }
  const int fr = lane & 15, fg = lane >> 4;
  constexpr int MB = 4;
  static_assert(MF % MB == 0, "MF must be a multiple of the batch");
  int nb[NF], nbc[NF];
  float4v bias4[NF];
#pragma unroll
  for (int nf = 0; nf < NF; ++nf) {
    nb[nf] = n_base + L::col(nf) + fg * L::LW;
    nbc[nf] = nb[nf] < p.N ? nb[nf] : p.N - 4;
    bias4[nf] = (ADD && p.bias) ? *(const float4v*)(p.bias + nbc[nf]) : float4v{0.f, 0.f, 0.f, 0.f};
  }
  if (ADD) F3R_EPI_WAIT_LOADS();
  if (EPI == F3R_EPI_GENERIC || EPI == F3R_EPI_CONVT) {
#pragma unroll
    for (int mb = 0; mb < MF; mb += MB) {
      int64_t m[MB], mc[MB];
#pragma unroll
      for (int i = 0; i < MB; ++i) {
        m[i] = m_base + L::row(mb + i) + fr;
        mc[i] = m[i] < p.M ? m[i] : p.M - 1;
      }
      float4v add[MB][NF];
      if (EPI == F3R_EPI_GENERIC && ADD) {
#pragma unroll
        for (int i = 0; i < MB; ++i)
#pragma unroll
          for (int nf = 0; nf < NF; ++nf) add[i][nf] = float4v{0.f, 0.f, 0.f, 0.f};
        gemm_additive_terms<T, NF, MB>(p, mc, nbc, [&](int i, int nf, float4v v) { add[i][nf] += v; });
        F3R_EPI_WAIT_LOADS();
      }
#pragma unroll
      for (int i = 0; i < MB; ++i) {
        if (m[i] >= p.M) continue;
        int64_t ct_base = 0;
        if (EPI == F3R_EPI_CONVT) {
          const int hw = p.ct_h * p.ct_w;
          const int b = (int)(m[i] / hw);
          const int rem = (int)(m[i] % hw);
          const int y = rem / p.ct_w, x = rem % p.ct_w;
          ct_base = (((int64_t)b * p.ct_h * p.ct_s + (int64_t)y * p.ct_s) * ((int64_t)p.ct_w * p.ct_s) + (int64_t)x * p.ct_s);
        }
#pragma unroll
        for (int nf = 0; nf < NF; ++nf) {
          if (nb[nf] >= p.N) continue;
          float4v v = acc[nf * MF + mb + i] + bias4[nf];
          if (p.act == F3R_ACT_GELU) {
            v[0] = gelu_erf(v[0]); v[1] = gelu_erf(v[1]); v[2] = gelu_erf(v[2]); v[3] = gelu_erf(v[3]);
          } else if (p.act == F3R_ACT_RELU) {
            v[0] = fmaxf(v[0], 0.f); v[1] = fmaxf(v[1], 0.f); v[2] = fmaxf(v[2], 0.f); v[3] = fmaxf(v[3], 0.f);
          }
          if (EPI == F3R_EPI_GENERIC) {
            if (ADD) v += add[i][nf];
            if (p.out_f32) *(float4v*)(p.out_f32 + m[i] * p.ldo_f32 + nb[nf]) = v;
            if (p.out_lp)
              store4_split<T>((uint16_t*)p.out_lp + m[i] * p.ldo_lp + nb[nf],
                              p.out_lp_lo ? (uint16_t*)p.out_lp_lo + m[i] * p.ldo_lp + nb[nf] : nullptr, v);
            if (p.out_f8) storeN_f8<1>((char*)p.out_f8 + m[i] * p.N * 2 + nb[nf], (char*)p.out_f8 + m[i] * p.N * 2 + p.N + nb[nf], &v);
            if (p.out_relu || p.out_relu_f8) {
              const float4v r = {fmaxf(v[0], 0.f), fmaxf(v[1], 0.f), fmaxf(v[2], 0.f), fmaxf(v[3], 0.f)};
              if (p.out_relu)
                store4_split<T>((uint16_t*)p.out_relu + m[i] * p.ldo_lp + nb[nf],
                                p.out_relu_lo ? (uint16_t*)p.out_relu_lo + m[i] * p.ldo_lp + nb[nf] : nullptr, r);
              if (p.out_relu_f8) storeN_f8<1>((char*)p.out_relu_f8 + m[i] * p.N * 2 + nb[nf], (char*)p.out_relu_f8 + m[i] * p.N * 2 + p.N + nb[nf], &r);
            }
          } else {
            const int tap = nb[nf] / p.ct_cout;
            const int co = nb[nf] - tap * p.ct_cout;
            const int dy = tap / p.ct_s, dx = tap - dy * p.ct_s;
            const int64_t pix = ct_base + (int64_t)dy * ((int64_t)p.ct_w * p.ct_s) + dx;
            store4_split<T>((uint16_t*)p.out_lp + pix * p.ct_cout + co, p.out_lp_lo ? (uint16_t*)p.out_lp_lo + pix * p.ct_cout + co : nullptr, v);
          }
        }
      }
    }
  } else {
    static_assert(EPI != F3R_EPI_QKV || (L::NG % 2 == 0 && NF % 2 == 0), "RoPE pairs need an even number of fragments per column group");
    const int Dq = p.qkv_dq ? p.qkv_dq : p.N / 3;
    const int Dkv = (p.N - Dq) / 2;
    const int part = n_base < Dq ? 0 : 1;
    const int Dm = part == 0 ? Dq : Dkv;
    const int col0 = part == 0 ? 0 : Dq;
    uint16_t* dst = (uint16_t*)(part == 0 ? p.q : p.k);
    const float qs = (part == 0 && p.q_scale != 0.f) ? p.q_scale : 1.f;
#pragma unroll
    for (int mb = 0; mb < MF; mb += MB) {
      int64_t m[MB];
      float4v c[MB][NF / 2], sn[MB][NF / 2];
#pragma unroll
      for (int i = 0; i < MB; ++i) {
        m[i] = m_base + L::row(mb + i) + fr;
        if (p.rope_cos) {
          const int64_t mc = m[i] < p.M ? m[i] : p.M - 1;
          const int pos = (int)(mc % p.seq_len);
          const int py = pos / p.rope_w, px = pos - py * p.rope_w;
          const int64_t grp = mc / p.rope_w;
#pragma unroll
          for (int j = 0; j < NF / 2; ++j) {
            const int h = ((n_base + L::col(2 * j)) >> 5) & 1;
            const int64_t toff = p.rope_mode == 1 ? grp * 32 + h * 16 : (int64_t)(h == 0 ? py : px) * 16;
            c[i][j] = *(const float4v*)(p.rope_cos + toff + fg * 4);
            sn[i][j] = *(const float4v*)(p.rope_sin + toff + fg * 4);
          }
        }
      }
      if (p.rope_cos) F3R_EPI_WAIT_LOADS();
#pragma unroll
      for (int i = 0; i < MB; ++i) {
        if (m[i] >= p.M) continue;
        float4v v[NF];
#pragma unroll
        for (int nf = 0; nf < NF; ++nf) v[nf] = acc[nf * MF + mb + i] + bias4[nf];
        if (p.rope_cos) {
#pragma unroll
          for (int j = 0; j < NF / 2; ++j) {
            const float4v a = v[2 * j], b = v[2 * j + 1];
            v[2 * j] = a * c[i][j] - b * sn[i][j];
            v[2 * j + 1] = b * c[i][j] + a * sn[i][j];
          }
        }
#pragma unroll
        for (int nf = 0; nf < NF; ++nf) store4_split<T>(dst + m[i] * (int64_t)Dm + (nb[nf] - col0), nullptr, v[nf] * qs);
      }
    }
  }
}

template <class T, class L, bool BIAS>
__device__ __forceinline__ void gemm_epilogue_vt(const f3r_gemm_args& p, const float4v* acc, int64_t m_base, int n_base, int lane) {
  constexpr int NF = L::NF, MF = L::MF;
  const int fr = lane & 15, fg = lane >> 4;
  const int Dq = p.qkv_dq ? p.qkv_dq : p.N / 3;
  const int Dm = (p.N - Dq) / 2;
  uint16_t* vt = (uint16_t*)p.vt;
  const bool vec_ok = ((p.seq_len | p.ldvt) & 3) == 0;
  if (!BIAS && vec_ok && p.M <= 0x7fffffffll && gemm_wave_interior<L>(p, m_base, n_base)) {
    const uint32_t seq = (uint32_t)p.seq_len;
    int64_t A[MF], B[NF];
#pragma unroll
    for (int mf = 0; mf < MF; ++mf) {
      const uint32_t mb = (uint32_t)(m_base + L::row(mf)) + (uint32_t)(fg * 4);
      const uint32_t sq = mb / seq, t = mb - sq * seq;
      A[mf] = (int64_t)sq * Dm * p.ldvt + t;
    }
#pragma unroll
    for (int nf = 0; nf < NF; ++nf) B[nf] = (int64_t)(n_base + L::col(nf) + fr - Dq - Dm) * p.ldvt;
#pragma unroll
    for (int nf = 0; nf < NF; ++nf)
#pragma unroll
      for (int mf = 0; mf < MF; ++mf) store4_split<T>(vt + A[mf] + B[nf], nullptr, acc[mf * NF + nf]);
    return;
  }
#pragma unroll
  for (int nf = 0; nf < NF; ++nf) {
    const int n = n_base + L::col(nf) + fr;
    const int d = n - Dq - Dm;
    const float bb = (BIAS && p.bias) ? p.bias[n] : 0.f;
#pragma unroll
    for (int mf = 0; mf < MF; ++mf) {
      const int64_t mb = m_base + L::row(mf) + fg * 4;
      if (mb >= p.M) continue;
      const float4v v = acc[mf * NF + nf] + bb;
      if (vec_ok) {
        const int64_t s = mb / p.seq_len, t = mb % p.seq_len;
        store4_split<T>(vt + (s * Dm + d) * p.ldvt + t, nullptr, v);
      } else {
#pragma unroll
        for (int j = 0; j < 4; ++j) {
          const int64_t m = mb + j;
          if (m < p.M) {
            const int64_t s = m / p.seq_len, t = m % p.seq_len;
            vt[(s * Dm + d) * p.ldvt + t] = to_lp<T>(v[j]);
          }
        }
      }
    }
  }
}

template <class T, class L>
__device__ __forceinline__ void gemm_epilogue_fin(const f3r_gemm_args& p, const float4v* acc, int64_t m0_tile, int wm, int wn, int lane, int tid,
                                                  float* scratch ) {
  static_assert(L::NF == 2 && L::MF == 8 && L::PAIRED, "fin epilogue: the 256 x 128 tile's paired fragment layout");
  const int fr = lane & 15, fg = lane >> 4;
  const int c0 = wn * 32 + fg * 8;
  float w[4][8];
#pragma unroll
  for (int o = 0; o < 4; ++o) {
    const float4v w0 = *(const float4v*)(p.fin_w + o * p.N + c0), w1 = *(const float4v*)(p.fin_w + o * p.N + c0 + 4);
#pragma unroll
    for (int j = 0; j < 4; ++j) { w[o][j] = w0[j]; w[o][4 + j] = w1[j]; }
  }
  const bool relu = p.act == F3R_ACT_RELU;
  float s[8][4];
#pragma unroll
  for (int mf = 0; mf < 8; ++mf) {
    float v[8];
#pragma unroll
    for (int j = 0; j < 4; ++j) { v[j] = acc[0 * 8 + mf][j]; v[4 + j] = acc[1 * 8 + mf][j]; }
    if (relu) {
#pragma unroll
      for (int j = 0; j < 8; ++j) v[j] = fmaxf(v[j], 0.f);
    }
#pragma unroll
    for (int o = 0; o < 4; ++o) {
      float a = v[0] * w[o][0];
#pragma unroll
      for (int j = 1; j < 8; ++j) a = __builtin_fmaf(v[j], w[o][j], a);
      s[mf][o] = a;
    }
  }
  const bool up32 = fg >= 2, up16 = (fg & 1) != 0;
  float t[4][4], u[2][4];
#pragma unroll
  for (int k = 0; k < 4; ++k)
#pragma unroll
    for (int o = 0; o < 4; ++o) {
      const float keep = up32 ? s[k + 4][o] : s[k][o], send = up32 ? s[k][o] : s[k + 4][o];
      t[k][o] = keep + __shfl_xor(send, 32, 64);
    }
#pragma unroll
  for (int k = 0; k < 2; ++k)
#pragma unroll
    for (int o = 0; o < 4; ++o) {
      const float keep = up16 ? t[k + 2][o] : t[k][o], send = up16 ? t[k][o] : t[k + 2][o];
      u[k][o] = keep + __shfl_xor(send, 16, 64);
    }
#pragma unroll
  for (int k = 0; k < 2; ++k) {
    const int mf = (up32 ? 4 : 0) + (up16 ? 2 : 0) + k;
    const int row = wm * 64 + (mf >> 2) * 128 + (mf & 3) * 16 + fr;
    *(float4v*)(scratch + (wn * 256 + row) * 4) = float4v{u[k][0], u[k][1], u[k][2], u[k][3]};
  }
  __syncthreads();
  if (tid < 256) {
    const int64_t pix = m0_tile + tid;
    float4v a = *(const float4v*)(scratch + tid * 4);
#pragma unroll
    for (int q = 1; q < 4; ++q) a += *(const float4v*)(scratch + (q * 256 + tid) * 4);
    if (pix < p.M) {
      const float a0 = a[0] + p.fin_b[0], a1 = a[1] + p.fin_b[1], a2 = a[2] + p.fin_b[2], a3 = p.fin_n_out > 3 ? a[3] + p.fin_b[3] : 0.f;
      float sc = 1.f;
      if (p.fin_depth_mode != 1 ) {
        const float d = sqrtf(a0 * a0 + a1 * a1 + a2 * a2);
        sc = (p.fin_depth_mode == 0  ? expm1f(d) : d * d) / fmaxf(d, 1e-8f);
      }
      p.fin_pts[pix * 3 + 0] = a0 * sc;
      p.fin_pts[pix * 3 + 1] = a1 * sc;
      p.fin_pts[pix * 3 + 2] = a2 * sc;
      if (p.fin_conf)
        p.fin_conf[pix] = p.fin_conf_mode == 0  ? p.fin_vmin + fminf(expf(a3), p.fin_vmax - p.fin_vmin)
                                                                  : (p.fin_vmax - p.fin_vmin) * (1.f / (1.f + expf(-a3))) + p.fin_vmin;
    }
  }
  __syncthreads();
}
```

Measured before the change: 36.12.

## Stage 3x3 conv inputs as 16x16 pixel-block halos in LDS for 256-tile GEMM

Adds a halo staging path for stride-1 fp16 3x3 convolutions in the 256-tile implicit GEMM. Each M tile becomes a 16x16 output pixel block, and its 18x18 input halo is loaded into LDS once per channel slice. All nine taps then read shifted windows from that halo, so the A operand is no longer fetched per tap through the offset table. The epilogues and residual init gain block-aware row mapping, and the path is used only when the block padding waste stays bounded. It adds kernel_sel 8 to opt out, and it raises LDS use and code complexity.

```diff
diff --git a/fast3r_amd/csrc/f3r_gemm.hip b/fast3r_amd/csrc/f3r_gemm.hip
--- a/fast3r_amd/csrc/f3r_gemm.hip
+++ b/fast3r_amd/csrc/f3r_gemm.hip
@@ -322,7 +322,7 @@
   if (a.split == F3R_SPLIT_X3F8)
     F3R_REQUIRE(a.a_mode == F3R_A_CONV3X3 && a.dtype == F3R_F16 && a.conv_C % 128 == 0 && a.w_scale && (((uintptr_t)a.w_scale) & 3) == 0,
                 "f3r_gemm: X3F8 needs a 3x3 convolution with conv_C %% 128 == 0 (got %d), fp16 planes and w_scale", a.conv_C);
-  F3R_REQUIRE((a.kernel_sel >= 0 && a.kernel_sel <= 7) || a.kernel_sel == 9 || a.kernel_sel >= 16, "f3r_gemm: bad kernel_sel %d", a.kernel_sel);
+  F3R_REQUIRE((a.kernel_sel >= 0 && a.kernel_sel <= 9) || a.kernel_sel >= 16, "f3r_gemm: bad kernel_sel %d", a.kernel_sel);
   F3R_REQUIRE(a.N % 4 == 0, "f3r_gemm: N %d must be a multiple of 4", a.N);
   F3R_REQUIRE(al16(a.A) && al16(a.W), "f3r_gemm: A/W must be 16-byte aligned");
   F3R_REQUIRE(a.dtype == F3R_F16 || a.dtype == F3R_BF16, "f3r_gemm: bad dtype %d", a.dtype);
@@ -390,7 +390,7 @@
     }
     return f3r_gemm256_launch(a, s, 1);
   }
-  if (a.kernel_sel == 6 || a.kernel_sel == 0 || a.kernel_sel == 9) {
+  if (a.kernel_sel == 6 || a.kernel_sel == 0 || a.kernel_sel == 8 || a.kernel_sel == 9) {
     const char* why = "";
     if (a.epi == F3R_EPI_QKV && f3r_gemm_asm_qkv_eligible(a, &why) && (a.kernel_sel == 6 || a.kernel_sel == 9 || f3r_gemm_asm_preferred((a.M / 256) * (a.N / 3 / 256))))
       return f3r_gemm_asm_qkv_launch(a, s);
@@ -401,7 +401,7 @@
     }
     if (ok && (a.kernel_sel == 6 || a.kernel_sel == 9 || f3r_gemm_asm_preferred((a.M / 256) * (a.N / 256)))) return f3r_gemm_asm_launch(a, s);
   }
-  const int sel = a.kernel_sel == 7 ? 0 : a.kernel_sel;
+  const int sel = (a.kernel_sel == 7 || a.kernel_sel == 8) ? 0 : a.kernel_sel;
   if (sel >= 2) F3R_REQUIRE(f3r_gemm256_eligible(a), "f3r_gemm: kernel_sel %d but the shape is not eligible for the 256-tile kernel", sel);
   if (sel >= 2 || (sel == 0 && f3r_gemm256_eligible(a) && f3r_gemm256_preferred(a))) return f3r_gemm256_launch(a, s, sel != 3);
   return a.dtype == F3R_F16 ? dispatch<F16>(a, s) : dispatch<BF16>(a, s);
diff --git a/fast3r_amd/csrc/f3r_gemm256.hip b/fast3r_amd/csrc/f3r_gemm256.hip
--- a/fast3r_amd/csrc/f3r_gemm256.hip
+++ b/fast3r_amd/csrc/f3r_gemm256.hip
@@ -18,6 +18,11 @@
     if (a.a_relu || a.conv_C % 64 != 0) return false;
     if (a.M / ((int64_t)a.conv_OH * a.conv_OW) * a.conv_H * a.conv_W * a.conv_C * 2 >= (1ll << 32)) return false;
     if (a.split == F3R_SPLIT_X3F8 && (a.conv_C % 128 != 0 || a.dtype != F3R_F16)) return false;
+    if (!f3r_conv_halo(a)) {
+      const int ct = a.conv_C / 64;
+      const int nk = a.split == F3R_SPLIT_X3F8 ? 18 * ct : (a.split == F3R_SPLIT_NONE ? 1 : a.split == F3R_SPLIT_W2 ? 2 : 3) * 9 * ct;
+      if (nk > TileCfg<1>::TAB_ENTRIES) return false;
+    }
   }
   if (a.split == F3R_SPLIT_X3F8 && a.a_mode != F3R_A_CONV3X3) return false;
   if (a.fin_w && (a.a_mode != F3R_A_CONV3X3 || a.N != 128 || a.epi != F3R_EPI_GENERIC)) return false;
diff --git a/fast3r_amd/csrc/f3r_gemm256_f8.hip b/fast3r_amd/csrc/f3r_gemm256_f8.hip
--- a/fast3r_amd/csrc/f3r_gemm256_f8.hip
+++ b/fast3r_amd/csrc/f3r_gemm256_f8.hip
@@ -18,10 +18,20 @@
 #endif
     if (a.dtype == F3R_BF16) return launch256<BF16, F3R_A_CONV3X3, F3R_EPI_GENERIC, 1, F3R_ADD_NONE, 1, false, true>(a, stream);
     if (f8 && a.kernel_sel == 5) return launch256<F16, F3R_A_CONV3X3, F3R_EPI_GENERIC, 1, F3R_ADD_NONE, 1, true, true, true>(a, stream);
+    if (f3r_conv_halo(a))
+      return f8 ? launch256<F16, F3R_A_CONV3X3, F3R_EPI_GENERIC, 1, F3R_ADD_NONE, 1, true, true, false, 0, true>(a, stream)
+                : launch256<F16, F3R_A_CONV3X3, F3R_EPI_GENERIC, 1, F3R_ADD_NONE, 1, false, true, false, 0, true>(a, stream);
     return f8 ? launch256<F16, F3R_A_CONV3X3, F3R_EPI_GENERIC, 1, F3R_ADD_NONE, 1, true, true>(a, stream)
               : launch256<F16, F3R_A_CONV3X3, F3R_EPI_GENERIC, 1, F3R_ADD_NONE, 1, false, true>(a, stream);
   }
   const int nh = tile_halves(a);
+  if (f3r_conv_halo(a)) {
+    if (add == F3R_ADD_RES_LP)
+      return nh == 2 ? launch256<F16, F3R_A_CONV3X3, F3R_EPI_GENERIC, 1, F3R_ADD_RES_LP, 2, true, false, false, 0, true>(a, stream)
+                     : launch256<F16, F3R_A_CONV3X3, F3R_EPI_GENERIC, 1, F3R_ADD_RES_LP, 1, true, false, false, 0, true>(a, stream);
+    return nh == 2 ? launch256<F16, F3R_A_CONV3X3, F3R_EPI_GENERIC, 1, F3R_ADD_NONE, 2, true, false, false, 0, true>(a, stream)
+                   : launch256<F16, F3R_A_CONV3X3, F3R_EPI_GENERIC, 1, F3R_ADD_NONE, 1, true, false, false, 0, true>(a, stream);
+  }
   if (add == F3R_ADD_RES_LP)
     return nh == 2 ? launch256<F16, F3R_A_CONV3X3, F3R_EPI_GENERIC, 1, F3R_ADD_RES_LP, 2, true>(a, stream)
                    : launch256<F16, F3R_A_CONV3X3, F3R_EPI_GENERIC, 1, F3R_ADD_RES_LP, 1, true>(a, stream);
diff --git a/fast3r_amd/csrc/f3r_gemm256_impl.h b/fast3r_amd/csrc/f3r_gemm256_impl.h
--- a/fast3r_amd/csrc/f3r_gemm256_impl.h
+++ b/fast3r_amd/csrc/f3r_gemm256_impl.h
@@ -1,5 +1,7 @@
 #pragma once
 #include <atomic>
+#include <type_traits>
+#include <utility>
 
 #include "f3r_common.h"
 #include "f3r_gemm_epi.h"
@@ -8,6 +10,10 @@
 namespace {
 
 constexpr int BM = 256, BK = 64, NT = 512;
+template <int V>
+struct IC {
+  static constexpr int value = V;
+};
 constexpr int HT = 128 * 64;
 template <int NH> struct TileCfg {
   static constexpr int BN = 128 * NH;
@@ -17,6 +23,32 @@
   static constexpr int LDS_BYTES = NBUF * BUF * 2 + TAB_ENTRIES * 16;
 };
 
+template <int NH> struct HaloCfg {
+  static constexpr int HINS = 41;
+  static constexpr int HPW = 6;
+  static constexpr int HB = HINS * 512;
+  static constexpr int WB = NH * HT;
+  static constexpr int NW = NH == 2 ? 2 : 3;
+  static constexpr int W0 = 2 * HB;
+  static constexpr int SINK = W0 + NW * WB;
+  static constexpr int LDS_BYTES = (SINK + 512) * 2;
+};
+inline bool f3r_conv_halo(const f3r_gemm_args& a) {
+  if (a.a_mode != F3R_A_CONV3X3 || a.conv_stride != 1 || a.dtype != F3R_F16 || a.kernel_sel == 8) return false;
+  if (a.split == F3R_SPLIT_X3F8 && a.N % 256 == 0) return false;
+  const int64_t blocks = (int64_t)((a.conv_OH + 15) / 16) * ((a.conv_OW + 15) / 16);
+  return blocks * 256 * 3 <= (int64_t)a.conv_OH * a.conv_OW * 4;
+}
+__host__ __device__ inline int64_t f3r_m_tiles(const f3r_gemm_args& a, bool halo) {
+  if (!halo) return (a.M + 255) / 256;
+  return a.M / ((int64_t)a.conv_OH * a.conv_OW) * ((a.conv_OH + 15) / 16) * ((a.conv_OW + 15) / 16);
+}
+
+template <class F, int... I>
+__device__ __forceinline__ void f3r_for_taps(F&& f, std::integer_sequence<int, I...>) {
+  (f(IC<I>{}), ...);
+}
+
 inline int f3r_num_cus() {
   constexpr int MAXD = 64;
   static std::atomic<int> cache[MAXD];
@@ -36,15 +68,12 @@
 typedef __attribute__((address_space(3))) void* lds_ptr_t;
 typedef const __attribute__((address_space(1))) void* glb_ptr_t;
 
-template <int V>
-struct IC {
-  static constexpr int value = V;
-};
 
 #define F3R_VMCNT(n) __builtin_amdgcn_s_waitcnt(0x0F70 | (n))
 #define F3R_LGKMCNT0() __builtin_amdgcn_s_waitcnt(0xC07F)
 
-template <class T, int A_MODE, int EPI, bool SWAP, int STAGGER, int ADDSRC, int NH = 2, int LAB = 0, bool F8 = false, bool FIN = false, bool MERGED = false>
+template <class T, int A_MODE, int EPI, bool SWAP, int STAGGER, int ADDSRC, int NH = 2, int LAB = 0, bool F8 = false, bool FIN = false, bool MERGED = false,
+          bool HALO = false>
 __device__ __forceinline__ void gemm256_body(const f3r_gemm_args& p, uint16_t* smem, const int64_t m0_tile, const int n0_tile, const bool first = true,
                                              const bool has_next = false, const int64_t m0_next = 0, const int n0_next = 0) {
   constexpr int BUF = TileCfg<NH>::BUF;
@@ -76,6 +105,8 @@
   const int ctiles8 = A_MODE == F3R_A_CONV3X3 ? p.conv_C / 128 : 1;
   static_assert(!F8 || (A_MODE == F3R_A_CONV3X3 && !SWAP), "fp8 correction segments: convolutions only");
   static_assert(!FIN || (NH == 1 && EPI == F3R_EPI_GENERIC && ADDSRC == 0 && !SWAP), "fused head tail: 256 x 128 tiles, no additive terms");
+  static_assert(!HALO || (A_MODE == F3R_A_CONV3X3 && EPI == F3R_EPI_GENERIC && !SWAP && !MERGED && LAB == 0), "halo staging: 3x3 convolutions");
+  typedef HaloCfg<NH> HC;
 
   uint32_t a_off[2][2], w_off[2][2];
   uint32_t a_msk[2][2];
@@ -84,9 +115,35 @@
   const uint32_t a_bytes = A_MODE == F3R_A_CONV3X3 ? (uint32_t)(p.M / ((int64_t)p.conv_OH * p.conv_OW) * p.conv_H * p.conv_W * p.conv_C * 2) : 0u;
   const char* Wb = nullptr;
   uint32_t wsc[NH][2];
+  uint32_t h_off[HaloCfg<NH>::HPW];
+  uint32_t h_msk = 0;
+  auto block_of = [&](int64_t tm0, int& b, int& y0, int& x0) {
+    const int nbx = (p.conv_OW + 15) >> 4, nby = (p.conv_OH + 15) >> 4;
+    const int64_t tm = tm0 >> 8;
+    b = (int)(tm / (nbx * nby));
+    const int rr = (int)(tm - (int64_t)b * (nbx * nby));
+    const int by = rr / nbx;
+    y0 = by * 16;
+    x0 = (rr - by * nbx) * 16;
+  };
   auto setup_tile = [&](int64_t tm0, int tn0) {
   m0 = tm0;
   n0 = tn0;
+  if constexpr (HALO) {
+    int b, y0, x0;
+    block_of(tm0, b, y0, x0);
+    h_msk = 0;
+#pragma unroll
+    for (int i = 0; i < HaloCfg<NH>::HPW; ++i) {
+      const int j = wid + 8 * i, q = j * 8 + (lane >> 3);
+      const int hy = q / 18, hx = q - hy * 18;
+      const int iy = y0 - 1 + hy, ix = x0 - 1 + hx;
+      const bool in = j < HaloCfg<NH>::HINS && q < 18 * 18 && iy >= 0 && iy < p.conv_H && ix >= 0 && ix < p.conv_W;
+      const int lc = (lane & 7) ^ ((hx >> 1) & 7);
+      h_off[i] = in ? (uint32_t)((((int64_t)b * p.conv_H + iy) * p.conv_W + ix) * p.conv_C * 2 + lc * 16) : 0u;
+      if (!in) h_msk |= 1u << i;
+    }
+  }
   Wb = (const char*)p.W + (int64_t)n0 * p.Kpad * 2;
   if constexpr (F8) {
 #pragma unroll
@@ -108,7 +165,10 @@
       if (n >= p.N) n = p.N - 1;
       w_off[h][i] = (uint32_t)(((int64_t)(n - n0) * p.Kpad + ((lane & 7) ^ w_key(r)) * 8) * 2);
       int64_t m = m0 + h * 128 + r;
-      if (A_MODE == F3R_A_PLAIN) {
+      if (HALO) {
+        a_off[h][i] = 0;
+        a_msk[h][i] = 0;
+      } else if (A_MODE == F3R_A_PLAIN) {
         if (m >= p.M) m = p.M - 1;
         a_off[h][i] = (uint32_t)(((m - m0) * p.lda + lc * 8) * 2);
         a_msk[h][i] = 0;
@@ -133,7 +193,7 @@
   };
   setup_tile(m0_tile, n0_tile);
 
-  constexpr bool TAB = A_MODE == F3R_A_CONV3X3;
+  constexpr bool TAB = A_MODE == F3R_A_CONV3X3 && !HALO;
   const int pix = TAB ? p.conv_C * 2 : 0;
   uint32_t* const tab = (uint32_t*)(smem + TileCfg<NH>::NBUF * BUF);
   if (TAB && first) {
@@ -439,14 +499,140 @@
 #undef F3R_MMA2_OPEN
 #undef F3R_MMA2_ISSUE
 #undef F3R_MMA2_CLOSE
+
+  struct HaloSlice {
+    const char* plane;
+    uint32_t adelta;
+    int wbase, wstr;
+    bool none;
+  };
+  auto halo_slice = [&](int s, int S) -> HaloSlice {
+    const bool none = s >= S;
+    if (none) s = S - 1;
+    if (F8 && s >= ctiles) {
+      const int u = s - ctiles, s8 = u / ctiles8, ct = u - s8 * ctiles8;
+      return HaloSlice{Alo, (uint32_t)((s8 == 1 ? p.conv_C : 0) + ct * 128), (s8 + 2) * Kpad1 + ct * 128, p.conv_C, none};
+    }
+    const int seg = s / ctiles, ct = s - seg * ctiles;
+    return HaloSlice{(!F8 && seg == 2) ? Alo : Ab, (uint32_t)(ct * 128), ((seg == 1 ? Kpad1 : 0) + ct * BK) * 2, 2 * p.conv_C, none};
+  };
+  auto issue_piece = [&](int i, const HaloSlice& sl, int hbuf) {
+    if (dry) return;
+    const int j = wid + 8 * i;
+    uint16_t* dst = smem + (j < HC::HINS ? hbuf + j * 512 : HC::SINK);
+    const __amdgpu_buffer_rsrc_t rs = __builtin_amdgcn_make_buffer_rsrc((void*)sl.plane, 0, a_bytes, 0x00020000);
+    const uint32_t inv = (((h_msk >> i) & 1u) || sl.none) ? 0xFFFFFFFFu : 0u;
+    __builtin_amdgcn_raw_ptr_buffer_load_lds(rs, (lds_ptr_t)dst, 16, (int)((h_off[i] + sl.adelta) | inv), 0, 0, 0);
+  };
+  auto hissue_w = [&](int h, int wbuf, int w_soff) {
+    if (dry) return;
+    uint16_t* dst = smem + wbuf + h * HT + wid * 2 * 8 * 64;
+    const __amdgpu_buffer_rsrc_t rs = __builtin_amdgcn_make_buffer_rsrc((void*)Wb, 0, 0x7fffffff, 0x00020000);
+#pragma unroll
+    for (int i = 0; i < 2; ++i)
+      __builtin_amdgcn_raw_ptr_buffer_load_lds(rs, (lds_ptr_t)(dst + i * 8 * 64), 16, (int)w_off[h][i], __builtin_amdgcn_readfirstlane(w_soff), 0, 0);
+  };
+  int h_rd[3][2];
+#pragma unroll
+  for (int dx = 0; dx < 3; ++dx)
+#pragma unroll
+    for (int ks = 0; ks < 2; ++ks) h_rd[dx][ks] = (wm * 4 * 18 + fr + dx) * 64 + (((ks * 4 + fg) ^ (((fr + dx) >> 1) & 7)) << 3);
+  auto hread_a = [&](auto e8, auto which, int hbo, int mh, int dy, int dx) {
+    const uint16_t* const hb = smem + hbo;
+    if constexpr (decltype(e8)::value) {
+      auto& g = decltype(which)::value ? ga1 : ga0;
+#pragma unroll
+      for (int mf = 0; mf < 4; ++mf) {
+        const u32x4 c0 = *(const u32x4*)(hb + h_rd[dx][0] + (mh * 8 + mf + dy) * 18 * 64);
+        const u32x4 c1 = *(const u32x4*)(hb + h_rd[dx][1] + (mh * 8 + mf + dy) * 18 * 64);
+        g[mf] = __builtin_shufflevector(c0, c1, 0, 1, 2, 3, 4, 5, 6, 7);
+      }
+    } else {
+      auto& f = decltype(which)::value ? fa1 : fa0;
+#pragma unroll
+      for (int ks = 0; ks < 2; ++ks)
+#pragma unroll
+        for (int mf = 0; mf < 4; ++mf) f[ks][mf] = as_vec8<T>(*(const u32x4*)(hb + h_rd[dx][ks] + (mh * 8 + mf + dy) * 18 * 64));
+    }
+  };
+  auto hread_w = [&](auto e8, int wbo) {
+    const uint16_t* const wb = smem + wbo;
+    if constexpr (decltype(e8)::value) {
+#pragma unroll
+      for (int nf = 0; nf < 2; ++nf) {
+        const u32x4 c0 = *(const u32x4*)(wb + w_rd[0] + nf * (PAIRED ? 4 : 16) * 64);
+        const u32x4 c1 = *(const u32x4*)(wb + w_rd[1] + nf * (PAIRED ? 4 : 16) * 64);
+        gw[nf] = __builtin_shufflevector(c0, c1, 0, 1, 2, 3, 4, 5, 6, 7);
+      }
+    } else {
+#pragma unroll
+      for (int ks = 0; ks < 2; ++ks)
+#pragma unroll
+        for (int nf = 0; nf < 2; ++nf) fw[ks][nf] = as_vec8<T>(*(const u32x4*)(wb + w_rd[ks] + nf * (PAIRED ? 4 : 16) * 64));
+    }
+  };
+  auto htap1 = [&](auto tapc, auto e8, int sa_shift, int sb, int hb, int hn, const HaloSlice& cur, const HaloSlice& nxt) {
+    constexpr int TP = decltype(tapc)::value, B = TP % 3, B2 = (TP + 2) % 3, DY = TP / 3, DX = TP % 3;
+    constexpr int HPW = HaloCfg<NH>::HPW;
+    constexpr int WAIT = 2 + (TP >= 1 && TP - 1 < HPW ? 1 : 0) + (TP < HPW ? 1 : 0);
+    hread_w(e8, HC::W0 + B * HC::WB);
+    __builtin_amdgcn_sched_barrier(0);
+    hread_a(e8, IC<0>{}, hb, 0, DY, DX);
+    hissue_w(0, HC::W0 + B2 * HC::WB, TP + 2 < 9 ? cur.wbase + (TP + 2) * cur.wstr : nxt.wbase + (TP - 7) * nxt.wstr);
+    F3R_PHASE_MMA(0, 0, 0)
+    hread_a(e8, IC<1>{}, hb, 1, DY, DX);
+    if constexpr (TP < HPW) issue_piece(TP, nxt, hn);
+    F3R_VMCNT(WAIT);
+    F3R_PHASE_MMA(1, 1, 0)
+  };
+  auto htap2 = [&](auto tapc, auto e8, int sa_shift, int sb, int hb, int hn, const HaloSlice& cur, const HaloSlice& nxt, int w_even, int w_odd) {
+    constexpr int TP = decltype(tapc)::value, DY = TP / 3, DX = TP % 3;
+    constexpr int HPW = HaloCfg<NH>::HPW;
+    constexpr int WAIT1 = 4 + (TP >= 1 && TP - 1 < HPW ? 1 : 0), WAIT3 = 4 + (TP < HPW ? 1 : 0);
+    const int wc = TP % 2 == 0 ? w_even : w_odd;
+    const int wo = TP % 2 == 0 ? w_odd : w_even;
+    hread_w(e8, wc);
+    __builtin_amdgcn_sched_barrier(0);
+    hread_a(e8, IC<0>{}, hb, 0, DY, DX);
+    F3R_PHASE_MMA(0, 0, 0)
+    hread_a(e8, IC<1>{}, hb, 1, DY, DX);
+    hissue_w(1, wo, TP + 1 < 9 ? cur.wbase + (TP + 1) * cur.wstr : nxt.wbase + (TP - 8) * nxt.wstr);
+    F3R_VMCNT(WAIT1);
+    F3R_PHASE_MMA(1, 1, 0)
+    hread_w(e8, wc + HT);
+    if constexpr (TP < HPW) issue_piece(TP, nxt, hn);
+    F3R_PHASE_MMA(1, 1, 1)
+    hissue_w(0, wc, TP + 2 < 9 ? cur.wbase + (TP + 2) * cur.wstr : nxt.wbase + (TP - 7) * nxt.wstr);
+    F3R_VMCNT(WAIT3);
+    F3R_PHASE_MMA(0, 0, 1)
+  };
 #undef F3R_PHASE_MMA
 
   typedef GemmFragLayout<2 * NH, 8, 2, 4, PAIRED> Frag;
-  const int64_t m_base = m0_tile + wm * 64;
+  int64_t m_base = m0_tile + wm * 64;
+  int64_t m_org = m0_tile;
+  GemmBlock bk_wave, bk_tile;
+  if constexpr (HALO) {
+    int b, y0, x0;
+    block_of(m0_tile, b, y0, x0);
+    m_org = ((int64_t)b * p.conv_OH + y0) * p.conv_OW + x0;
+    m_base = m_org + (int64_t)wm * 4 * p.conv_OW;
+    bk_tile = GemmBlock{p.conv_OW, p.conv_OH - y0, p.conv_OW - x0};
+    bk_wave = GemmBlock{p.conv_OW, p.conv_OH - y0 - wm * 4, p.conv_OW - x0};
+  }
   const int n_base = n0_tile + wn * 32;
   auto opening_loads = [&]() {
     a_seg = a_kk = a_t = 0;
     w_seg = w_kk = w_t = 0;
+    if constexpr (HALO) {
+      const HaloSlice s0 = halo_slice(0, nk / 9);
+#pragma unroll
+      for (int i = 0; i < HaloCfg<NH>::HPW; ++i) issue_piece(i, s0, 0);
+      hissue_w(0, HC::W0, s0.wbase);
+      if constexpr (NH == 2) hissue_w(1, HC::W0, s0.wbase);
+      hissue_w(0, HC::W0 + HC::WB, s0.wbase + s0.wstr);
+      return;
+    }
     if constexpr (NH == 2) {
       if (!dry) fetch();
       issue_a(0, 0);
@@ -480,8 +666,11 @@
   dry = !first;
   opening_loads();
   dry = false;
-  gemm_acc_init_additive<T, Frag, ADDSRC, SWAP>(p, acc, m_base, n_base, lane);
-  if (first && MERGED) {
+  gemm_acc_init_additive<T, Frag, ADDSRC, SWAP, HALO>(p, acc, m_base, n_base, lane, bk_wave);
+  if (first && HALO) {
+    if constexpr (NH == 2) F3R_VMCNT(4);
+    else F3R_VMCNT(2);
+  } else if (first && MERGED) {
     if constexpr (NH == 2) F3R_VMCNT(8);
     else F3R_VMCNT(6);
   } else if (first) {
@@ -504,7 +693,26 @@
     else tile1(bufc, e8, sa_shift, sb);
   };
   const int nk16 = F8 ? nk1 : nk;
-  if constexpr (NH == 2) {
+  if constexpr (HALO) {
+    const int S = nk / 9;
+    auto slice = [&](int s, auto e8, int sa_shift, int sb) {
+      const HaloSlice cur = halo_slice(s, S), nxt = halo_slice(s + 1, S);
+      const int hb = (s & 1) * HC::HB, hn = ((s + 1) & 1) * HC::HB;
+      if constexpr (NH == 2) {
+        const int w_even = HC::W0 + (s & 1) * HC::WB;
+        const int w_odd = HC::W0 + ((s & 1) ^ 1) * HC::WB;
+        f3r_for_taps([&](auto tapc) { htap2(tapc, e8, sa_shift, sb, hb, hn, cur, nxt, w_even, w_odd); }, std::make_integer_sequence<int, 9>{});
+      } else {
+        f3r_for_taps([&](auto tapc) { htap1(tapc, e8, sa_shift, sb, hb, hn, cur, nxt); }, std::make_integer_sequence<int, 9>{});
+      }
+    };
+    const int S16 = F8 ? ctiles : S;
+    for (int s = 0; s < S16; ++s) slice(s, E16{}, 0, 0);
+    if constexpr (F8) {
+      for (int s = S16; s < S16 + ctiles8; ++s) slice(s, E8{}, 0, 127);
+      for (int s = S16 + ctiles8; s < S; ++s) slice(s, E8{}, 8, 115);
+    }
+  } else if constexpr (NH == 2) {
     if (LAB) {
       tile(IC<0>{}, E16{}, 0, 0);
       if (nk > 1) tile(IC<1>{}, E16{}, 0, 0);
@@ -545,9 +753,9 @@
 
   if constexpr (FIN) {
     __builtin_amdgcn_s_barrier();
-    gemm_epilogue_fin<T, Frag>(p, acc, m0_tile, wm, wn, lane, tid, (float*)(smem + 2 * BUF));
+    gemm_epilogue_fin<T, Frag, HALO>(p, acc, m_org, wm, wn, lane, tid, (float*)(smem + (HALO ? HC::W0 + 2 * HC::WB : 2 * BUF)), bk_tile);
   } else if (SWAP) gemm_epilogue_vt<T, Frag, false>(p, acc, m_base, n_base, lane);
-  else gemm_epilogue_default<T, EPI, Frag, false>(p, acc, m_base, n_base, lane);
+  else gemm_epilogue_default<T, EPI, Frag, false, HALO>(p, acc, m_base, n_base, lane, bk_wave);
   if (LAB & 128) {
     __builtin_amdgcn_sched_barrier(0);
     stamp[3] = __builtin_amdgcn_s_memtime();
@@ -560,12 +768,13 @@
   }
 }
 
-template <class T, int A_MODE, int EPI, int STAGGER, int ADDSRC, int NH, bool F8 = false, bool FIN = false, bool MERGED = false, int LAB = 0>
+template <class T, int A_MODE, int EPI, int STAGGER, int ADDSRC, int NH, bool F8 = false, bool FIN = false, bool MERGED = false, int LAB = 0,
+          bool HALO = false>
 __global__ __launch_bounds__(NT, 1) void gemm256_kernel(const f3r_gemm_args p) {
   extern __shared__ __attribute__((aligned(16))) uint16_t smem[];
   constexpr int BN = TileCfg<NH>::BN;
   const int n_tiles_n = (p.N + BN - 1) / BN;
-  const int64_t n_tiles_m = (p.M + BM - 1) / BM;
+  const int64_t n_tiles_m = f3r_m_tiles(p, HALO);
   const int64_t n_wg = n_tiles_m * n_tiles_n;
   auto tile_of = [&](int64_t wg, int64_t& m0, int& n0) {
     {
@@ -598,21 +807,22 @@
         done = true;
       }
     }
-    if (!done) gemm256_body<T, A_MODE, EPI, false, STAGGER, ADDSRC, NH, LAB, F8, FIN, MERGED>(p, smem, m0, n0, first, has_next, m0n, n0n);
+    if (!done) gemm256_body<T, A_MODE, EPI, false, STAGGER, ADDSRC, NH, LAB, F8, FIN, MERGED, HALO>(p, smem, m0, n0, first, has_next, m0n, n0n);
     first = false;
   }
 }
 
-template <class T, int A_MODE, int EPI, int STAGGER, int ADDSRC, int NH, bool F8 = false, bool FIN = false, bool MERGED = false, int LAB = 0>
+template <class T, int A_MODE, int EPI, int STAGGER, int ADDSRC, int NH, bool F8 = false, bool FIN = false, bool MERGED = false, int LAB = 0,
+          bool HALO = false>
 int launch256(const f3r_gemm_args& a, hipStream_t stream) {
   static bool attr_set = false;
-  auto kern = gemm256_kernel<T, A_MODE, EPI, STAGGER, ADDSRC, NH, F8, FIN, MERGED, LAB>;
-  constexpr int LDS_BYTES = TileCfg<NH>::LDS_BYTES, BN = TileCfg<NH>::BN;
+  auto kern = gemm256_kernel<T, A_MODE, EPI, STAGGER, ADDSRC, NH, F8, FIN, MERGED, LAB, HALO>;
+  constexpr int LDS_BYTES = HALO ? HaloCfg<NH>::LDS_BYTES : TileCfg<NH>::LDS_BYTES, BN = TileCfg<NH>::BN;
   if (!attr_set) {
     (void)hipFuncSetAttribute((const void*)kern, hipFuncAttributeMaxDynamicSharedMemorySize, LDS_BYTES);
     attr_set = true;
   }
-  const int64_t tiles = ((a.M + BM - 1) / BM) * ((a.N + BN - 1) / BN);
+  const int64_t tiles = f3r_m_tiles(a, HALO) * ((a.N + BN - 1) / BN);
   const int64_t grid = (a.kernel_sel == 5 || tiles <= f3r_num_cus()) ? tiles : f3r_num_cus();
   hipLaunchKernelGGL(kern, dim3((unsigned)grid), dim3(NT), LDS_BYTES, stream, a);
   return f3r_check_launch("f3r_gemm(256)");
@@ -641,7 +851,17 @@
 #define F3R_L256(AM, EP, AD) (nh == 2 ? F3R_L256H(AM, EP, AD, 2) : F3R_L256H(AM, EP, AD, 1))
   const int add = gemm_additive_pattern(a);
   const int nh = tile_halves(a);
-  if (a.a_mode == F3R_A_CONV3X3) return add == F3R_ADD_RES_LP ? F3R_L256(F3R_A_CONV3X3, F3R_EPI_GENERIC, F3R_ADD_RES_LP) : F3R_L256(F3R_A_CONV3X3, F3R_EPI_GENERIC, F3R_ADD_NONE);
+  if (a.a_mode == F3R_A_CONV3X3) {
+    if constexpr (std::is_same<T, F16>::value) {
+      if (f3r_conv_halo(a)) {
+#define F3R_LHALO(AD) (nh == 2 ? launch256<T, F3R_A_CONV3X3, F3R_EPI_GENERIC, 1, AD, 2, false, false, false, 0, true>(a, stream) \
+                               : launch256<T, F3R_A_CONV3X3, F3R_EPI_GENERIC, 1, AD, 1, false, false, false, 0, true>(a, stream))
+        return add == F3R_ADD_RES_LP ? F3R_LHALO(F3R_ADD_RES_LP) : F3R_LHALO(F3R_ADD_NONE);
+#undef F3R_LHALO
+      }
+    }
+    return add == F3R_ADD_RES_LP ? F3R_L256(F3R_A_CONV3X3, F3R_EPI_GENERIC, F3R_ADD_RES_LP) : F3R_L256(F3R_A_CONV3X3, F3R_EPI_GENERIC, F3R_ADD_NONE);
+  }
   switch (a.epi) {
     case F3R_EPI_GENERIC:
       return add == F3R_ADD_RES_F32 ? F3R_L256(F3R_A_PLAIN, F3R_EPI_GENERIC, F3R_ADD_RES_F32)
diff --git a/fast3r_amd/csrc/f3r_gemm_epi.h b/fast3r_amd/csrc/f3r_gemm_epi.h
--- a/fast3r_amd/csrc/f3r_gemm_epi.h
+++ b/fast3r_amd/csrc/f3r_gemm_epi.h
@@ -12,6 +12,19 @@
   static __device__ __forceinline__ int col(int nf) { return (nf / NG) * 128 + (nf % NG) * (PAIRED_ ? 4 : 16); }
   static __device__ __forceinline__ int col_end() { return ((NF - 1) / NG) * 128 + NG * 16; }
 };
+
+struct GemmBlock {
+  int64_t pitch = 0;
+  int rows = 0, cols = 0;
+};
+template <class L, bool BLK>
+__device__ __forceinline__ int64_t frag_row(int64_t m_base, const GemmBlock& bk, int mf) {
+  return BLK ? m_base + (int64_t)(L::row(mf) >> 4) * bk.pitch : m_base + L::row(mf);
+}
+template <class L, bool BLK>
+__device__ __forceinline__ bool frag_row_ok(const f3r_gemm_args& p, int64_t m_base, const GemmBlock& bk, int mf, int fr) {
+  return BLK ? ((L::row(mf) >> 4) < bk.rows && fr < bk.cols) : m_base + L::row(mf) + fr < p.M;
+}
 
 __device__ __forceinline__ float gelu_erf(float x) {
   const float z = fabsf(x) * 0.70710678118654752440f;
@@ -165,8 +178,12 @@
   return a.rowadd ? F3R_ADD_ROWADD : (a.res_f32 ? F3R_ADD_RES_F32 : F3R_ADD_RES_LP);
 }
 
-template <class T, class L, int SRC, bool SWAP>
-__device__ __forceinline__ void gemm_acc_init_additive(const f3r_gemm_args& p, float4v* acc, int64_t m_base, int n_base, int lane) {
+template <class L, bool BLK = false>
+__device__ __forceinline__ bool gemm_wave_interior(const f3r_gemm_args& p, int64_t m_base, int n_base, const GemmBlock& bk = GemmBlock{});
+
+template <class T, class L, int SRC, bool SWAP, bool BLK = false>
+__device__ __forceinline__ void gemm_acc_init_additive(const f3r_gemm_args& p, float4v* acc, int64_t m_base, int n_base, int lane,
+                                                       const GemmBlock& bk = GemmBlock{}) {
   constexpr int NF = L::NF, MF = L::MF;
   const int fr = lane & 15, fg = lane >> 4;
   if (SWAP) {
@@ -179,7 +196,7 @@
     }
     return;
   }
-  if (SRC != F3R_ADD_ROWADD && m_base + L::row(MF - 1) + 16 <= p.M && n_base + L::col_end() <= p.N) {
+  if (SRC != F3R_ADD_ROWADD && gemm_wave_interior<L, BLK>(p, m_base, n_base, bk)) {
     float4v b4[NF];
 #pragma unroll
     for (int nf = 0; nf < NF; ++nf)
@@ -195,7 +212,7 @@
       const uint32_t off = (uint32_t)(fr * (int)p.ldr_f32 + fg * L::LW) * 4u;
 #pragma unroll
       for (int mf = 0; mf < MF; ++mf) {
-        const char* const row = (const char*)p.res_f32 + ((m_base + L::row(mf)) * p.ldr_f32 + n_base) * 4;
+        const char* const row = (const char*)p.res_f32 + (frag_row<L, BLK>(m_base, bk, mf) * p.ldr_f32 + n_base) * 4;
 #pragma unroll
         for (int nf = 0; nf < NF; ++nf) acc[nf * MF + mf] = *(const float4v*)(row + L::col(nf) * 4 + off);
       }
@@ -204,7 +221,7 @@
       const uint32_t off2 = (uint32_t)(fr * (int)p.ldr_lp2 + fg * L::LW) * 2u;
 #pragma unroll
       for (int mf = 0; mf < MF; ++mf) {
-        const int64_t ro = ((m_base + L::row(mf)) * p.ldr_lp + n_base) * 2;
+        const int64_t ro = (frag_row<L, BLK>(m_base, bk, mf) * p.ldr_lp + n_base) * 2;
 #pragma unroll
         for (int nf = 0; nf < NF; nf += L::STEP) {
           float4v t[L::STEP];
@@ -216,7 +233,7 @@
       if (p.res_lp_lo) {
 #pragma unroll
         for (int mf = 0; mf < MF; ++mf) {
-          const int64_t ro = ((m_base + L::row(mf)) * p.ldr_lp + n_base) * 2;
+          const int64_t ro = (frag_row<L, BLK>(m_base, bk, mf) * p.ldr_lp + n_base) * 2;
 #pragma unroll
           for (int nf = 0; nf < NF; nf += L::STEP) {
             float4v t[L::STEP];
@@ -229,7 +246,7 @@
       if (p.res_lp2) {
 #pragma unroll
         for (int mf = 0; mf < MF; ++mf) {
-          const int64_t ro = ((m_base + L::row(mf)) * p.ldr_lp2 + n_base) * 2;
+          const int64_t ro = (frag_row<L, BLK>(m_base, bk, mf) * p.ldr_lp2 + n_base) * 2;
 #pragma unroll
           for (int nf = 0; nf < NF; nf += L::STEP) {
             float4v t[L::STEP];
@@ -241,7 +258,7 @@
         if (p.res_lp2_lo) {
 #pragma unroll
           for (int mf = 0; mf < MF; ++mf) {
-            const int64_t ro = ((m_base + L::row(mf)) * p.ldr_lp2 + n_base) * 2;
+            const int64_t ro = (frag_row<L, BLK>(m_base, bk, mf) * p.ldr_lp2 + n_base) * 2;
 #pragma unroll
             for (int nf = 0; nf < NF; nf += L::STEP) {
             float4v t[L::STEP];
@@ -277,8 +294,12 @@
   int64_t mc[MF];
 #pragma unroll
   for (int mf = 0; mf < MF; ++mf) {
-    const int64_t m = m_base + L::row(mf) + fr;
-    mc[mf] = m < p.M ? m : p.M - 1;
+    if (BLK) {
+      mc[mf] = frag_row_ok<L, BLK>(p, m_base, bk, mf, fr) ? frag_row<L, BLK>(m_base, bk, mf) + fr : 0;
+    } else {
+      const int64_t m = m_base + L::row(mf) + fr;
+      mc[mf] = m < p.M ? m : p.M - 1;
+    }
   }
   if (SRC == F3R_ADD_RES_F32) {
 #pragma unroll
@@ -324,9 +345,10 @@
 
 #define F3R_EPI_WAIT_LOADS() __builtin_amdgcn_s_waitcnt(0x0F70)
 
-template <class L>
-__device__ __forceinline__ bool gemm_wave_interior(const f3r_gemm_args& p, int64_t m_base, int n_base) {
-  return m_base + L::row(L::MF - 1) + 16 <= p.M && n_base + L::col_end() <= p.N;
+template <class L, bool BLK>
+__device__ __forceinline__ bool gemm_wave_interior(const f3r_gemm_args& p, int64_t m_base, int n_base, const GemmBlock& bk) {
+  const bool rows = BLK ? ((L::row(L::MF - 1) >> 4) < bk.rows && bk.cols >= 16) : m_base + L::row(L::MF - 1) + 16 <= p.M;
+  return rows && n_base + L::col_end() <= p.N;
 }
 
 template <int V>
@@ -334,8 +356,9 @@
   static constexpr int value = V;
 };
 
-template <class T, class L>
-__device__ __forceinline__ void gemm_epilogue_generic_interior(const f3r_gemm_args& p, const float4v* acc, int64_t m_base, int n_base, int lane) {
+template <class T, class L, bool BLK = false>
+__device__ __forceinline__ void gemm_epilogue_generic_interior(const f3r_gemm_args& p, const float4v* acc, int64_t m_base, int n_base, int lane,
+                                                               const GemmBlock& bk = GemmBlock{}) {
   constexpr int NF = L::NF, MF = L::MF;
   const int fr = lane & 15, fg = lane >> 4;
   const uint32_t off_f32 = (uint32_t)(fr * (int)p.ldo_f32 + fg * L::LW) * 4u;
@@ -346,7 +369,7 @@
     constexpr int ACT = decltype(act_c)::value, KIND = decltype(kind_c)::value;
 #pragma unroll
     for (int mf = 0; mf < MF; ++mf) {
-      const int64_t mrow = m_base + L::row(mf);
+      const int64_t mrow = frag_row<L, BLK>(m_base, bk, mf);
       char* const bf = (KIND >= 2 && p.out_f32) ? (char*)p.out_f32 + (mrow * p.ldo_f32 + n_base) * 4 : nullptr;
       const int64_t lp_row = (mrow * p.ldo_lp + n_base) * 2;
       char* const bl = (KIND != 2 && p.out_lp) ? (char*)p.out_lp + lp_row : nullptr;
@@ -445,12 +468,14 @@
   }
 }
 
-template <class T, int EPI, class L, bool ADD>
-__device__ __forceinline__ void gemm_epilogue_default(const f3r_gemm_args& p, const float4v* acc, int64_t m_base, int n_base, int lane) {
+template <class T, int EPI, class L, bool ADD, bool BLK = false>
+__device__ __forceinline__ void gemm_epilogue_default(const f3r_gemm_args& p, const float4v* acc, int64_t m_base, int n_base, int lane,
+                                                      const GemmBlock& bk = GemmBlock{}) {
   constexpr int NF = L::NF, MF = L::MF;
+  static_assert(!BLK || (EPI == F3R_EPI_GENERIC && !ADD), "pixel-block rows: the generic epilogue of the 256-tile kernel");
   if constexpr (!ADD && EPI != F3R_EPI_CONVT) {
-    if (gemm_wave_interior<L>(p, m_base, n_base) && p.M <= 0x7fffffffll) {
-      if constexpr (EPI == F3R_EPI_GENERIC) gemm_epilogue_generic_interior<T, L>(p, acc, m_base, n_base, lane);
+    if (gemm_wave_interior<L, BLK>(p, m_base, n_base, bk) && p.M <= 0x7fffffffll) {
+      if constexpr (EPI == F3R_EPI_GENERIC) gemm_epilogue_generic_interior<T, L, BLK>(p, acc, m_base, n_base, lane, bk);
       else gemm_epilogue_qk_interior<T, L>(p, acc, m_base, n_base, lane);
       return;
     }
@@ -471,9 +496,11 @@
 #pragma unroll
     for (int mb = 0; mb < MF; mb += MB) {
       int64_t m[MB], mc[MB];
+      bool ok[MB];
 #pragma unroll
       for (int i = 0; i < MB; ++i) {
-        m[i] = m_base + L::row(mb + i) + fr;
+        ok[i] = frag_row_ok<L, BLK>(p, m_base, bk, mb + i, fr);
+        m[i] = BLK ? (ok[i] ? frag_row<L, BLK>(m_base, bk, mb + i) + fr : 0) : m_base + L::row(mb + i) + fr;
         mc[i] = m[i] < p.M ? m[i] : p.M - 1;
       }
       float4v add[MB][NF];
@@ -487,7 +514,7 @@
       }
 #pragma unroll
       for (int i = 0; i < MB; ++i) {
-        if (m[i] >= p.M) continue;
+        if (!ok[i]) continue;
         int64_t ct_base = 0;
         if (EPI == F3R_EPI_CONVT) {
           const int hw = p.ct_h * p.ct_w;
@@ -633,9 +660,9 @@
   }
 }
 
-template <class T, class L>
+template <class T, class L, bool BLK = false>
 __device__ __forceinline__ void gemm_epilogue_fin(const f3r_gemm_args& p, const float4v* acc, int64_t m0_tile, int wm, int wn, int lane, int tid,
-                                                  float* scratch ) {
+                                                  float* scratch , const GemmBlock& bk = GemmBlock{}) {
   static_assert(L::NF == 2 && L::MF == 8 && L::PAIRED, "fin epilogue: the 256 x 128 tile's paired fragment layout");
   const int fr = lane & 15, fg = lane >> 4;
   const int c0 = wn * 32 + fg * 8;
@@ -689,11 +716,11 @@
   }
   __syncthreads();
   if (tid < 256) {
-    const int64_t pix = m0_tile + tid;
+    const int64_t pix = BLK ? m0_tile + (int64_t)(tid >> 4) * bk.pitch + (tid & 15) : m0_tile + tid;
     float4v a = *(const float4v*)(scratch + tid * 4);
 #pragma unroll
     for (int q = 1; q < 4; ++q) a += *(const float4v*)(scratch + (q * 256 + tid) * 4);
-    if (pix < p.M) {
+    if (BLK ? ((tid >> 4) < bk.rows && (tid & 15) < bk.cols) : pix < p.M) {
       const float a0 = a[0] + p.fin_b[0], a1 = a[1] + p.fin_b[1], a2 = a[2] + p.fin_b[2], a3 = p.fin_n_out > 3 ? a[3] + p.fin_b[3] : 0.f;
       float sc = 1.f;
       if (p.fin_depth_mode != 1 ) {
```

New measurement: 36.26 (median of 6 runs). No clear change (+0.4%).
